# bkainz/fetalReconstruction

Measured on AMD Instinct MI355X. Metric: MVoxels/s per SR iteration (PSF fwd+back), 4-stack 1.0mm SVR, 1/2/4/8 GPU, higher is better.
Workload: dtype f32

## Files before the change

fetalreconstruction_amd/csrc/svr_cell.inc:

```

struct CellRec {
  short cx, cl, cz;
  unsigned short dead;
  float bx, by, bz;
  float f0, f1;
  uint32_t idx;
};
static_assert(sizeof(CellRec) == 32, "CellRec layout");

struct CellRun {
  uint32_t start, count;
  uint32_t cell, slice;
  short czmin, czmax;
  unsigned short n[4];
  int pad;
};
static_assert(sizeof(CellRun) == 32, "CellRun layout");

struct CellClass {
  int x0, l0;
  int ncx, ncl;
  int pfirst, plast;
  int ng;
  int cell_base;
// ... 384 lines not shown
  const uint32_t quad = item >> 10;
  const int ci = quad >= (uint32_t)ca.cls[1].cell_base ? 1 : 0;
  const CellClass &C = ca.cls[ci];
  const int P = C.pfirst + (int)(item & 1023u);
  const bool swap = ci == 0;
  const int vgy = swap ? vg.vz : vg.vy;
  const int lq = (int)quad - C.cell_base;
  const int ql = lq / C.ncx, qx = lq - ql * C.ncx;
  const int cx0 = C.x0 + qx * ca.CX, cl0 = C.l0 + ql * ca.CL;
  const int PL = ca.PL, PP = ca.PP;
  const bool idle = lane >= CH;
  const int slot = idle ? NSLOT - 1 : lane / SL, y = lane % SL;
  const float fyl = (float)(y - NC);
  const int lox = cx0 - NC, loy = cl0 - NC;
  f2 *pb = box + slot * PP - lox;
  for (int i = lane; i < NSLOT * PP; i += 64) box[i] = (f2){0.0f, 0.0f};
  __syncthreads();

  const uint32_t rfirst = ent.z, r1 = ent.w;
  uint32_t nreach = 0;
  for (uint32_t rb = rfirst; rb < r1; rb += 64) {
    CellRun Rl;
    Rl.start = Rl.count = Rl.slice = 0u;
    bool hit = false;
    if (rb + lane < r1) {
      Rl = ca.runs[rb + lane];
      hit = Rl.czmin - NC <= P && Rl.czmax + NH >= P;
    }
    unsigned long long todo = __ballot(hit);
    if (nparts > 1u) {
      const uint32_t ord = nreach + (uint32_t)__popcll(todo & ((1ull << lane) - 1ull));
      nreach += (uint32_t)__popcll(todo);
      todo = __ballot(hit && ord % nparts == rep);
    }
    const int mine = idle ? 0x7fffffff : NSLOT * y + slot;
    CellRec nrec;
    uint32_t npid = 0u;
    bool nact = false;
    nrec.f0 = nrec.f1 = 0.0f; nrec.cz = 0; nrec.dead = 0;
    auto request_run = [&](int rl) {
      const uint32_t st = (uint32_t)__builtin_amdgcn_readlane((int)Rl.start, rl), cn = (uint32_t)__builtin_amdgcn_readlane((int)Rl.count, rl);
      if ((uint32_t)mine < cn) {
        nrec = ca.recs[st + (uint32_t)mine];
        if (COEFF) npid = ca.pid[st + (uint32_t)mine];
        if (COEFF == 3) nact = ca.act[st + (uint32_t)mine] != 0;
      }
    };
    if (todo) request_run((int)__builtin_ctzll(todo));
    while (todo) {
      const int rl = (int)__builtin_ctzll(todo);
      todo &= todo - 1ull;
      const uint32_t sl = (uint32_t)__builtin_amdgcn_readlane((int)Rl.slice, rl);
      const uint32_t rstart = (uint32_t)__builtin_amdgcn_readlane((int)Rl.start, rl), rcount = (uint32_t)__builtin_amdgcn_readlane((int)Rl.count, rl);
      const SliceConst &S = a.sc[sl];
      const RowConst RC = load_row_const(S);
      for (uint32_t c0 = 0; c0 < rcount; c0 += CH) {
        CellRec r0;
        bool act0 = false;
        int pid0 = 0;
        if (c0 + (uint32_t)mine < rcount) {
          bool on0 = nact;
          if (c0 == 0) { r0 = nrec; pid0 = (int)npid; }
          else {
            r0 = ca.recs[rstart + c0 + (uint32_t)mine];
            if (COEFF) pid0 = (int)ca.pid[rstart + c0 + (uint32_t)mine];
            if (COEFF == 3) on0 = ca.act[rstart + c0 + (uint32_t)mine] != 0;
          }
          act0 = (COEFF == 3 ? on0 : (r0.f0 != 0.0f || r0.f1 != 0.0f)) && r0.cz - NC <= P && r0.cz + NH >= P;
        }
        if (c0 + CH >= rcount && todo) request_run((int)__builtin_ctzll(todo));
        if (ca.dbg == 2 && lane == 0) atomicAdd(ca.stats + 0, 1ull);
        if (!__any(act0)) continue;
        const bool dead0 = act0 && !PVR && ((r0.dead >> (P - r0.cz + NC)) & 1u);
        const int sh = SL * slot;
        unsigned ml = idle ? 0u : (unsigned)(__ballot(act0 && !dead0) >> sh) & ((1u << SL) - 1u);
        unsigned md = idle ? 0u : (unsigned)(__ballot(dead0) >> sh) & ((1u << SL) - 1u);
        if (ca.dbg == 2) {
          int mx = __popc(ml);
          for (int o = 16; o < 64; o <<= 1) mx = max(mx, __shfl_xor(mx, o, 64));
          if (y == 0 && !idle) { atomicAdd(ca.stats + 3, (unsigned long long)__popc(ml)); atomicAdd(ca.stats + 4, (unsigned long long)__popc(md)); }
          if (lane == 0) { atomicAdd(ca.stats + 1, 1ull); atomicAdd(ca.stats + 2, (unsigned long long)mx); }
        }
        const int w0a = (int)((unsigned short)r0.cx | ((unsigned)(unsigned short)r0.cl << 16));
        struct Unit { int cx, cy, cz; float bx, by, bz, f0, f1; int pid; };
        auto fetch = [&](int j) -> Unit {
          const int src = slot * SL + (j & 15);
          Unit u;
          const int w0 = __shfl(w0a, src, 64);
          u.cx = (int)(short)(w0 & 0xFFFF); u.cy = w0 >> 16;
          u.cz = __shfl((int)r0.cz, src, 64);
          u.f0 = __shfl(r0.f0, src, 64); u.f1 = __shfl(r0.f1, src, 64);
          u.pid = COEFF ? __shfl(pid0, src, 64) : 0;
          u.bx = u.by = u.bz = 0.0f;
          return u;
        };
        auto fetch_b = [&](int j, Unit &u) {
          const int src = slot * SL + (j & 15);
          u.bx = __shfl(r0.bx, src, 64); u.by = __shfl(r0.by, src, 64); u.bz = __shfl(r0.bz, src, 64);
        };
        if (ca.dbg == 0) {
          if (COEFF == 1) {
            constexpr int RING = SVR_CELL_RING;
            float4 ring[RING][NS / 4];
            Unit ru[RING];
            bool rv[RING];
            auto request = [&](Unit &u, bool &valid, float4 (&dst)[NS / 4]) {
              valid = ml != 0u;
              const int j = valid ? __builtin_ctz(ml) : 0;
              ml &= ml - 1u;
              u = fetch(j);
              if (valid) {
                const float4 *src = a.coeff + ((size_t)(uint32_t)u.pid * NS + (size_t)(P - u.cz + NC)) * (NS / 4 * 16) + (y < NS ? y : 0);
#pragma unroll
                for (int q = 0; q < NS / 4; ++q) dst[q] = load_stream(src + q * 16);
              }
            };
#pragma unroll
            for (int r3 = 0; r3 < RING; ++r3) request(ru[r3], rv[r3], ring[r3]);
            while (__any(rv[0])) {
#pragma unroll
              for (int r3 = 0; r3 < RING; ++r3) {
                if (!__any(rv[r3])) break;
                const Unit u = ru[r3];
                const bool valid = rv[r3];
                const int ay = u.cy + y - NC;
                const bool rowok = valid && y < NS && ay < vgy;
                const int rbx = rowok ? (ay - loy) * PL + u.cx - NC : lox;
                constexpr int PARTS = NS == 16 ? 2 : 1, PT = NS / PARTS;
                static_assert(PT % 4 == 0, "whole float4 per part");
                const f2 ff = (f2){u.f0, u.f1};
#pragma unroll
                for (int hq = 0; hq < PARTS; ++hq) {
                  f2 acc[PT];
#pragma unroll
                  for (int x = 0; x < PT; ++x) acc[x] = pb[rbx + hq * PT + x];
                  if (rowok) {
#pragma unroll
                    for (int q = 0; q < PT / 4; ++q) {
                      const float4 c = ring[r3][hq * (PT / 4) + q];
                      pb[rbx + hq * PT + 4 * q] = fma2(bc2(c.x), ff, acc[4 * q]);
                      pb[rbx + hq * PT + 4 * q + 1] = fma2(bc2(c.y), ff, acc[4 * q + 1]);
                      pb[rbx + hq * PT + 4 * q + 2] = fma2(bc2(c.z), ff, acc[4 * q + 2]);
                      pb[rbx + hq * PT + 4 * q + 3] = fma2(bc2(c.w), ff, acc[4 * q + 3]);
                    }
                  }
                }
                request(ru[r3], rv[r3], ring[r3]);
              }
            }
          } else {
            bool nvalid = ml != 0u;
            int jn = nvalid ? __builtin_ctz(ml) : 0;
            ml &= ml - 1u;
            Unit un = fetch(jn);
            fetch_b(jn, un);
            while (__any(nvalid)) {
              const bool valid = nvalid;
              const Unit u = un;
              nvalid = ml != 0u;
              jn = nvalid ? __builtin_ctz(ml) : 0;
              ml &= ml - 1u;
              un = fetch(jn);
              fetch_b(jn, un);
              const float fzu = (float)(P - u.cz);
              const int ay = u.cy + y - NC;
              const bool rowok = valid && y < NS && ay < vgy;
              const int rbx = rowok ? (ay - loy) * PL + u.cx - NC : lox;
              float out[NS];
              eval_row_t<NS, PVR, true, SVR_CELL_EVAL_H(NS)>(RC, u.bx, u.by, u.bz, swap ? fzu : fyl, swap ? fyl : fzu, out);
              if (COEFF == 3) {
                if (valid && y < NS) {
                  float4 *dstp = const_cast<float4 *>(a.coeff) + ((size_t)(uint32_t)u.pid * NS + (size_t)(P - u.cz + NC)) * (NS / 4 * 16) + y;
#pragma unroll
                  for (int q = 0; q < NS / 4; ++q) store_stream(dstp + q * 16, out[4 * q], out[4 * q + 1], out[4 * q + 2], out[4 * q + 3]);
                }
              }
              f2 acc[NS];
#pragma unroll
              for (int x = 0; x < NS; ++x) acc[x] = pb[rbx + x];
              if (rowok) {
                const f2 ff = (f2){u.f0, u.f1};
#pragma unroll
                for (int x = 0; x < NS; ++x) acc[x] = fma2(bc2(out[x]), ff, acc[x]);
#pragma unroll
                for (int x = 0; x < NS; ++x) pb[rbx + x] = acc[x];
              }
            }
          }
          if (!PVR) {
            while (__any(md != 0u)) {
              const bool va = md != 0u;
              const int ja = va ? __builtin_ctz(md) : 0;
              md &= md - 1u;
              const bool vb = md != 0u;
              const int jb = vb ? __builtin_ctz(md) : 0;
              md &= md - 1u;
              Unit Ra = fetch(ja), Rb = fetch(jb);
              fetch_b(ja, Ra); fetch_b(jb, Rb);
              const float fua = (float)(P - Ra.cz), fub = (float)(P - Rb.cz);
              const float fya = swap ? fua : fyl, fza = swap ? fyl : fua, fyb = swap ? fub : fyl, fzb = swap ? fyl : fub;
              const f2 rowx = (f2){__builtin_fmaf(RC.Lp[1], fya, __builtin_fmaf(RC.Lp[2], fza, Ra.bx)),
                                   __builtin_fmaf(RC.Lp[1], fyb, __builtin_fmaf(RC.Lp[2], fzb, Rb.bx))};
              const f2 rowy = (f2){__builtin_fmaf(RC.Lp[4], fya, __builtin_fmaf(RC.Lp[5], fza, Ra.by)),
                                   __builtin_fmaf(RC.Lp[4], fyb, __builtin_fmaf(RC.Lp[5], fzb, Rb.by))};
              const f2 rowz = (f2){__builtin_fmaf(RC.Lp[7], fya, __builtin_fmaf(RC.Lp[8], fza, Ra.bz)),
                                   __builtin_fmaf(RC.Lp[7], fyb, __builtin_fmaf(RC.Lp[8], fzb, Rb.bz))};
              f2 xs[1], ys[1], t0[1];
              xs[0] = fma2(bc2(RC.Lp[0]), bc2((float)(-NC)), rowx);
              ys[0] = fma2(bc2(RC.Lp[3]), bc2((float)(-NC)), rowy);
              eval_pairs_xyz<1, false>(RC, xs, ys, t0);
              const f2 v = t0[0] * gauss_first_tap2<NC>(RC, rowz);
              const int aya = Ra.cy + y - NC, ayb = Rb.cy + y - NC;
              if (va && aya < vgy) {
                f2 *q = pb + (aya - loy) * PL + Ra.cx - NC;
                *q = fma2(bc2(v.x), (f2){Ra.f0, Ra.f1}, *q);
              }
              if (vb && ayb < vgy) {
                f2 *q = pb + (ayb - loy) * PL + Rb.cx - NC;
                *q = fma2(bc2(v.y), (f2){Rb.f0, Rb.f1}, *q);
              }
            }
          }
        }
      }
    }
  }
  __syncthreads();
  f2 *dst = ca.stage + (size_t)bid * (size_t)PP;
  for (int i = lane; i < PP; i += 64) {
    f2 v = (box[i] + box[PP + i]) + (box[2 * PP + i] + box[3 * PP + i]);
    if (NSLOT == 5) v = v + box[4 * PP + i];
    dst[i] = v;
  }
  if (ca.trace && lane == 0) {
    unsigned hw, xcc;
    asm volatile("s_getreg_b32 %0, hwreg(HW_REG_HW_ID)" : "=s"(hw));
    asm volatile("s_getreg_b32 %0, hwreg(HW_REG_XCC_ID)" : "=s"(xcc));
    ca.trace[3 * (size_t)bid] = t_start;
    ca.trace[3 * (size_t)bid + 1] = __builtin_amdgcn_s_memrealtime();
    ca.trace[3 * (size_t)bid + 2] = (unsigned long long)hw | (unsigned long long)xcc << 32;
  }
}

__device__ __forceinline__ f2 combine_class(const CellArgs &ca, const CellClass &C, int c, int x, int y, int z, int NC, int NH, f2 acc) {
  const int Pv = c == 0 ? y : z, Lv = c == 0 ? z : y;
  const int pa = Pv > 0 ? Pv : min(C.pfirst, 0), pe = Pv > 0 ? Pv : 0;
  const int la = Lv > 0 ? Lv : min(C.l0 - NC, 0), le = Lv > 0 ? Lv : 0;
  const int xa = x > 0 ? x : min(C.x0 - NC, 0), xe = x > 0 ? x : 0;
  for (int Ps = max(pa, C.pfirst); Ps <= min(pe, C.plast); ++Ps) {
    const int g = Ps - C.pfirst;
    for (int Ls = la; Ls <= le; ++Ls) {
      const int jlo = max(-floordiv(-(Ls - C.l0 - NH - (ca.CL - 1)), ca.CL), 0);
      const int jhi = min(floordiv(Ls - C.l0 + NC, ca.CL), C.ncl * ca.QL - 1);
      for (int Xs = xa; Xs <= xe; ++Xs) {
        const int ilo = max(-floordiv(-(Xs - C.x0 - NH - (ca.CX - 1)), ca.CX), 0);
// ... 197 lines not shown
  const float fyl = (float)(y - NC);
  SlotSum<SL> ssum;
  ssum.init(lane);
  {
    const uint32_t sty = swap ? (uint32_t)(vg.vx * vg.vy) : (uint32_t)vg.vx, stz = swap ? (uint32_t)vg.vx : (uint32_t)(vg.vx * vg.vy);
    const uint32_t zoff = sat0(P) * stz;
    RowWalk w;
    w.init(lane, 64, PL);
    for (int i = lane; i < PP; i += 64, w.step()) {
      const int gx = w.x + lox, gy = w.y + loy;
      f2 v = (f2){0.0f, 0.0f};
      if (gx < vg.vx && gy < vgy) {
        const uint32_t vi = sat0(gx) + sat0(gy) * sty + zoff;
        if (G1) {
          v = (f2){1.0f, a.mask[vi] != 0.0f ? 1.0f : 0.0f};
        } else if (!PVR || a.volm) {
          const float2 t = a.volm[vi];
          v = (f2){t.x, t.y};
        } else {
          const float m = a.mask[vi] != 0.0f ? 1.0f : 0.0f;
          const int X = (int)sat0(gx), L = (int)sat0(gy), Z = (int)sat0(P);
          v = (f2){m != 0.0f ? pvr_tex(a.vol, vg, X, swap ? Z : L, swap ? L : Z) : 0.0f, m};
        }
      }
      box[i] = v;
    }
  }
  __syncthreads();
  const f2 *pb = box - lox;
  const float4 *stage = reinterpret_cast<const float4 *>(tile + 2 * ((PP + 1) & ~1)) + lane;
  const uint32_t stage_lds = COEFF == 2 ? (uint32_t)__builtin_amdgcn_readfirstlane((int)lds_addr_of(tile + 2 * ((PP + 1) & ~1))) : 0u;

  const uint32_t rfirst = ent.z, r1 = ent.w;
  uint32_t nreach = 0;
  for (uint32_t rb = rfirst; rb < r1; rb += 64) {
    CellRun Rl;
    Rl.start = Rl.count = Rl.slice = 0u;
    bool hit = false;
    if (rb + lane < r1) {
      Rl = ca.runs[rb + lane];
      hit = Rl.czmin - NC <= P && Rl.czmax + NH >= P;
    }
    unsigned long long todo = __ballot(hit);
    if (nparts > 1u) {
      const uint32_t ord = nreach + (uint32_t)__popcll(todo & ((1ull << lane) - 1ull));
      nreach += (uint32_t)__popcll(todo);
      todo = __ballot(hit && ord % nparts == rep);
    }
    const int mine = idle ? 0x7fffffff : NSLOT * y + slot;
    CellRec nrec;
    float ngf = 0.0f;
    uint32_t npid = 0u;
    nrec.cz = 0; nrec.dead = 0;
    auto request_run = [&](int rl) {
      const uint32_t st = (uint32_t)__builtin_amdgcn_readlane((int)Rl.start, rl), cn = (uint32_t)__builtin_amdgcn_readlane((int)Rl.count, rl);
      if ((uint32_t)mine < cn) { nrec = ca.recs[st + (uint32_t)mine]; ngf = G1 ? 1.0f : gf[st + (uint32_t)mine]; if (COEFF) npid = ca.pid[st + (uint32_t)mine]; }
    };
    if (todo) request_run((int)__builtin_ctzll(todo));
    while (todo) {
      const int rl = (int)__builtin_ctzll(todo);
      todo &= todo - 1ull;
      const uint32_t sl = (uint32_t)__builtin_amdgcn_readlane((int)Rl.slice, rl);
      const uint32_t rstart = (uint32_t)__builtin_amdgcn_readlane((int)Rl.start, rl), rcount = (uint32_t)__builtin_amdgcn_readlane((int)Rl.count, rl);
      const SliceConst &S = a.sc[sl];
      const RowConst RC = load_row_const(S);
      for (uint32_t c0 = 0; c0 < rcount; c0 += CH) {
        CellRec r0;
        float g0 = 0.0f;
        bool act0 = false;
        int pid0 = 0;
        if (c0 + (uint32_t)mine < rcount) {
          if (c0 == 0) { r0 = nrec; g0 = ngf; pid0 = (int)npid; }
          else { r0 = ca.recs[rstart + c0 + (uint32_t)mine]; g0 = G1 ? 1.0f : gf[rstart + c0 + (uint32_t)mine]; if (COEFF) pid0 = (int)ca.pid[rstart + c0 + (uint32_t)mine]; }
          act0 = g0 != 0.0f && r0.cz - NC <= P && r0.cz + NH >= P;
        }
        if (c0 + CH >= rcount && todo) request_run((int)__builtin_ctzll(todo));
        if (!__any(act0)) continue;
        const bool dead0 = act0 && !PVR && ((r0.dead >> (P - r0.cz + NC)) & 1u);
        const int sh = SL * slot;
        unsigned ml = idle ? 0u : (unsigned)(__ballot(act0 && !dead0) >> sh) & ((1u << SL) - 1u);
        unsigned md = idle ? 0u : (unsigned)(__ballot(dead0) >> sh) & ((1u << SL) - 1u);
        const int w0a = (int)((unsigned short)r0.cx | ((unsigned)(unsigned short)r0.cl << 16));
        const uint32_t myrec = rstart + c0 + (uint32_t)mine;
        struct Unit { int cx, cy, cz; float bx, by, bz; uint32_t rec; int pid; };
        auto fetch = [&](int j) -> Unit {
          const int src = slot * SL + (j & 15);
          Unit u;
          const int w0 = __shfl(w0a, src, 64);
          u.cx = (int)(short)(w0 & 0xFFFF); u.cy = w0 >> 16;
          u.cz = __shfl((int)r0.cz, src, 64);
          u.bx = __shfl(r0.bx, src, 64); u.by = __shfl(r0.by, src, 64); u.bz = __shfl(r0.bz, src, 64);
          u.rec = (uint32_t)__shfl((int)myrec, src, 64);
          u.pid = COEFF ? __shfl(pid0, src, 64) : 0;
          return u;
        };
        if (COEFF == 2) {
          static_assert(COEFF != 2 || NS == 16, "the landing stages are laid out for support 16");
          constexpr int DD = SVR_CELL_DMA_DEPTH, HQ = NS / 4;
          unsigned mli = ml;
          int s_issue = 0, s_use = 0;
          auto issue = [&]() -> bool {
            const bool vi = mli != 0u;
            if (!__any(vi)) return false;
            const int j = vi ? __builtin_ctz(mli) : 0;
            mli &= mli - 1u;
            const int src = slot * SL + (j & 15);
            const int pid = __shfl(pid0, src, 64), czk = __shfl((int)r0.cz, src, 64);
            const float4 *srcp = vi ? a.coeff + ((size_t)(uint32_t)pid * NS + (size_t)(P - czk + NC)) * (HQ * 16) + y : a.coeff + lane;
            const uint32_t dst = stage_lds + (uint32_t)s_issue * (HQ * 1024u);
#pragma unroll
            for (int q = 0; q < HQ; ++q) glds16(srcp + q * 16, dst + q * 1024u);
            s_issue = s_issue + 1 == DD ? 0 : s_issue + 1;
            return true;
          };
#pragma unroll
          for (int k = 0; k < DD - 1; ++k) issue();
          bool nvalid = ml != 0u;
          int jn = nvalid ? __builtin_ctz(ml) : 0;
          ml &= ml - 1u;
          Unit un = fetch(jn);
          while (__any(nvalid)) {
            const bool ahead = issue();
            const bool valid = nvalid;
            const Unit u = un;
            nvalid = ml != 0u;
            jn = nvalid ? __builtin_ctz(ml) : 0;
            ml &= ml - 1u;
            un = fetch(jn);
            const int ay = u.cy + y - NC;
            const bool rowok = valid && ay < vgy;
            f2 acc = (f2){0.0f, 0.0f};
            {
              const f2 *q = pb + (rowok ? (ay - loy) * PL + u.cx - NC : lox);
              if (ahead) glds_wait<(DD - 1) * HQ>(); else glds_wait<0>();
              const float4 *st = stage + s_use * (HQ * 64);
              s_use = s_use + 1 == DD ? 0 : s_use + 1;
#pragma unroll
              for (int qq = 0; qq < HQ; ++qq) {
                const float4 c = st[qq * 64];
                acc = fma2(bc2(c.x), q[4 * qq], acc);
                acc = fma2(bc2(c.y), q[4 * qq + 1], acc);
                acc = fma2(bc2(c.z), q[4 * qq + 2], acc);
                acc = fma2(bc2(c.w), q[4 * qq + 3], acc);
              }
            }
            if (!rowok) acc = (f2){0.0f, 0.0f};
            acc.x = ssum.sum(acc.x); acc.y = ssum.sum(acc.y);
            if (valid && y == 0) part[(size_t)(P - u.cz + NC) * npart + u.rec] = acc;
          }
        } else if (COEFF == 1) {
          constexpr int RING = SVR_CELL_RING;
          float4 ring[RING][NS / 4];
          Unit ru[RING];
          bool rv[RING];
          auto request = [&](Unit &u, bool &valid, float4 (&dst)[NS / 4]) {
            valid = ml != 0u;
            const int j = valid ? __builtin_ctz(ml) : 0;
            ml &= ml - 1u;
            u = fetch(j);
            if (valid) {
              const float4 *src = a.coeff + ((size_t)(uint32_t)u.pid * NS + (size_t)(P - u.cz + NC)) * (NS / 4 * 16) + (y < NS ? y : 0);
#pragma unroll
              for (int q = 0; q < NS / 4; ++q) dst[q] = load_stream(src + q * 16);
            }
          };
#pragma unroll
          for (int r3 = 0; r3 < RING; ++r3) request(ru[r3], rv[r3], ring[r3]);
          while (__any(rv[0])) {
#pragma unroll
            for (int r3 = 0; r3 < RING; ++r3) {
              if (!__any(rv[r3])) break;
              const Unit u = ru[r3];
              const bool valid = rv[r3];
              const int ay = u.cy + y - NC;
              const bool rowok = valid && y < NS && ay < vgy;
              f2 acc = (f2){0.0f, 0.0f};
              {
                const f2 *q = pb + (rowok ? (ay - loy) * PL + u.cx - NC : lox);
#pragma unroll
                for (int qq = 0; qq < NS / 4; ++qq) {
                  const float4 c = ring[r3][qq];
                  acc = fma2(bc2(c.x), q[4 * qq], acc);
                  acc = fma2(bc2(c.y), q[4 * qq + 1], acc);
                  acc = fma2(bc2(c.z), q[4 * qq + 2], acc);
                  acc = fma2(bc2(c.w), q[4 * qq + 3], acc);
                }
              }
              request(ru[r3], rv[r3], ring[r3]);
              if (!rowok) acc = (f2){0.0f, 0.0f};
              acc.x = ssum.sum(acc.x); acc.y = ssum.sum(acc.y);
              if (valid && y == 0) part[(size_t)(P - u.cz + NC) * npart + u.rec] = acc;
            }
          }
        }
        if (COEFF == 0 || COEFF == 3) {
        bool nvalid = ml != 0u;
        int jn = nvalid ? __builtin_ctz(ml) : 0;
        ml &= ml - 1u;
        Unit un = fetch(jn);
        while (__any(nvalid)) {
          const bool valid = nvalid;
          const Unit u = un;
          nvalid = ml != 0u;
          jn = nvalid ? __builtin_ctz(ml) : 0;
          ml &= ml - 1u;
          un = fetch(jn);
          const float fzu = (float)(P - u.cz);
          const int ay = u.cy + y - NC;
          const bool rowok = valid && y < NS && ay < vgy;
          float out[NS];
          eval_row_t<NS, PVR, true, SVR_CELL_EVAL_H_FWD(NS)>(RC, u.bx, u.by, u.bz, swap ? fzu : fyl, swap ? fyl : fzu, out);
          if (COEFF == 3) {
            if (valid && y < NS) {
              float4 *dstp = const_cast<float4 *>(a.coeff) + ((size_t)(uint32_t)u.pid * NS + (size_t)(P - u.cz + NC)) * (NS / 4 * 16) + y;
#pragma unroll
              for (int q = 0; q < NS / 4; ++q) store_stream(dstp + q * 16, out[4 * q], out[4 * q + 1], out[4 * q + 2], out[4 * q + 3]);
            }
          }
          f2 acc = (f2){0.0f, 0.0f};
          double accd = 0.0;
          bool hit = false;
          {
            const f2 *q = pb + (rowok ? (ay - loy) * PL + u.cx - NC : lox);
            f2 v[NS];
#pragma unroll
            for (int x = 0; x < NS; ++x) v[x] = q[x];
#pragma unroll
            for (int x = 0; x < NS; ++x) {
              if (G1) {
                accd += (double)(out[x] * v[x].x);
                hit = hit | ((v[x].y != 0.0f) & (__float_as_uint(out[x]) != 0x80000000u));
              } else {
                acc = fma2(bc2(out[x]), v[x], acc);
              }
            }
          }
          if (G1) {
            if (!rowok) { accd = 0.0; hit = false; }
            accd = ssum.sum(accd);
            const bool anyhit = idle ? false : (((uint32_t)(__ballot(hit) >> (SL * slot)) & ((1u << SL) - 1u)) != 0u);
            if (valid && y == 0) partd[(size_t)(P - u.cz + NC) * npart + u.rec] = anyhit ? -accd : accd;
          } else {
            if (!rowok) acc = (f2){0.0f, 0.0f};
            acc.x = ssum.sum(acc.x); acc.y = ssum.sum(acc.y);
            if (valid && y == 0) part[(size_t)(P - u.cz + NC) * npart + u.rec] = acc;
          }
        }
        }
        if (!PVR) {
          while (__any(md != 0u)) {
            const bool va = md != 0u;
            const int ja = va ? __builtin_ctz(md) : 0;
            md &= md - 1u;
            const bool vb = md != 0u;
            const int jb = vb ? __builtin_ctz(md) : 0;
            md &= md - 1u;
            const Unit Ra = fetch(ja), Rb = fetch(jb);
            const float fua = (float)(P - Ra.cz), fub = (float)(P - Rb.cz);
            const float fya = swap ? fua : fyl, fza = swap ? fyl : fua, fyb = swap ? fub : fyl, fzb = swap ? fyl : fub;
            const f2 rowx = (f2){__builtin_fmaf(RC.Lp[1], fya, __builtin_fmaf(RC.Lp[2], fza, Ra.bx)),
                                 __builtin_fmaf(RC.Lp[1], fyb, __builtin_fmaf(RC.Lp[2], fzb, Rb.bx))};
            const f2 rowy = (f2){__builtin_fmaf(RC.Lp[4], fya, __builtin_fmaf(RC.Lp[5], fza, Ra.by)),
                                 __builtin_fmaf(RC.Lp[4], fyb, __builtin_fmaf(RC.Lp[5], fzb, Rb.by))};
            const f2 rowz = (f2){__builtin_fmaf(RC.Lp[7], fya, __builtin_fmaf(RC.Lp[8], fza, Ra.bz)),
                                 __builtin_fmaf(RC.Lp[7], fyb, __builtin_fmaf(RC.Lp[8], fzb, Rb.bz))};
            f2 xs[1], ys[1], t0[1];
            xs[0] = fma2(bc2(RC.Lp[0]), bc2((float)(-NC)), rowx);
            ys[0] = fma2(bc2(RC.Lp[3]), bc2((float)(-NC)), rowy);
            eval_pairs_xyz<1, false>(RC, xs, ys, t0);
            const f2 v = t0[0] * gauss_first_tap2<NC>(RC, rowz);
            const int aya = Ra.cy + y - NC, ayb = Rb.cy + y - NC;
            f2 wa = (f2){0.0f, 0.0f}, wb = (f2){0.0f, 0.0f};
            if (va && aya < vgy) wa = pb[(aya - loy) * PL + Ra.cx - NC];
            if (vb && ayb < vgy) wb = pb[(ayb - loy) * PL + Rb.cx - NC];
            f2 acca = bc2(v.x) * wa, accb = bc2(v.y) * wb;
            if (G1) {
              double da = row_sum16((double)acca.x), db = row_sum16((double)accb.x);
              const bool anya = ((uint32_t)(__ballot(wa.y != 0.0f) >> (16 * slot)) & 0xFFFFu) != 0u;
              const bool anyb = ((uint32_t)(__ballot(wb.y != 0.0f) >> (16 * slot)) & 0xFFFFu) != 0u;
              if (y == 0) {
                if (va) partd[(size_t)(P - Ra.cz + NC) * npart + Ra.rec] = anya ? -da : da;
                if (vb) partd[(size_t)(P - Rb.cz + NC) * npart + Rb.rec] = anyb ? -db : db;
              }
            } else {
              acca.x = row_sum16(acca.x); acca.y = row_sum16(acca.y);
              accb.x = row_sum16(accb.x); accb.y = row_sum16(accb.y);
              if (y == 0) {
                if (va) part[(size_t)(P - Ra.cz + NC) * npart + Ra.rec] = acca;
                if (vb) part[(size_t)(P - Rb.cz + NC) * npart + Rb.rec] = accb;
              }
            }
          }
        }
      }
    }
  }
}
// ... 540 lines not shown
```

fetalreconstruction_amd/csrc/svr_hip.hip:

```cpp
#include <hip/hip_runtime.h>
#include <float.h>
#include <limits.h>
#include <math.h>
#include <stdint.h>
#include <stdio.h>
#include <string.h>

#include <algorithm>
#include <chrono>
#include <string>
#include <vector>

#include "../../include/svr_hip.h"

int svr_sort_keys_u64(void *tmp, size_t *tmp_bytes, const uint64_t *keys_in, uint64_t *keys_out, size_t n, int end_bit, hipStream_t stream);
int svr_inclusive_sum_u32(void *tmp, size_t *tmp_bytes, const uint32_t *in, uint32_t *out, size_t n, hipStream_t stream);

#define SVR_STEP 0.0001f
#define PSF_SUPPORT 16
#define PSF_CENTRE 7
#define PSF_EPS_F 0.00001f
#define LDS_ROW 20
#define WAVES_PER_BLOCK 4
#define CHUNK_PIX 2048
// ... 18 lines not shown
  float I2W[12];
  float T[12];
  float A[12];
  float Lp[9];
  float dim[3];
  float kx, ky, inv2s2;
  float dd, w;
  int own;
  float invD;
  float pad[9];
};
static_assert(sizeof(SliceConst) == 256, "SliceConst layout");

struct VolGeom {
  int vx, vy, vz;
  float W2I[12];
  float c0[3];
  int pvr;
};

__host__ __device__ __forceinline__ float canon_exp_neg(float a) {
  const float LOG2E = 1.442695040888963407359924681001892137426645954152985934135449406931f;
  const float L2U = 0.693145751953125f;
  const float L2L = 1.428606765330187045e-06f;
  float d = -a;
  float q = __builtin_rintf(d * LOG2E);
  float s = __builtin_fmaf(q, -L2U, d);
  s = __builtin_fmaf(q, -L2L, s);
  float u = 0.000198527617612853646278381f;
  u = __builtin_fmaf(u, s, 0.00139304355252534151077271f);
  u = __builtin_fmaf(u, s, 0.00833336077630519866943359f);
  u = __builtin_fmaf(u, s, 0.0416664853692054748535156f);
  u = __builtin_fmaf(u, s, 0.166666671633720397949219f);
  u = __builtin_fmaf(u, s, 0.5f);
  u = __builtin_fmaf(s * s, u, s) + 1.0f;
  float r = ldexpf(u, (int)q);
  return (a > 87.0f) ? 0.0f : r;
}
__device__ __forceinline__ float wave_sum(float v) {
#pragma unroll
  for (int o = 32; o > 0; o >>= 1) v += __shfl_xor(v, o, 64);
  return v;
}
__device__ __forceinline__ double wave_sum(double v) {
#pragma unroll
  for (int o = 32; o > 0; o >>= 1) v += __shfl_xor(v, o, 64);
  return v;
}

__device__ __forceinline__ void matvec3(const float *M, float x, float y, float z, float &a,
                                        float &b, float &c) {
  a = M[0] * x + M[1] * y + M[2] * z + M[3];
  b = M[4] * x + M[5] * y + M[6] * z + M[7];
  c = M[8] * x + M[9] * y + M[10] * z + M[11];
}

enum { MODE_GAUSS = 0, MODE_FWD = 1, MODE_BACK = 2, MODE_BIAS = 3 };

struct PsfArgs {
  const SliceConst *sc;
  VolGeom vg;
  int sx, sy;
  const uint32_t *list;
  uint32_t n;
  const float *slices;
  const float *mask;
  float *psf_sums;
  const float *scales;
  const float *bias;
  const unsigned char *flag;
  unsigned char *flag_out;
  const unsigned char *spx;
  float *recon, *volw;
  int *voxcount;
  const float *vol;
  const float2 *volm;
  float *simslices, *simweights;
  unsigned char *siminside;
  unsigned char *slice_inside;
  const float *weights, *slice_weights;
  float *addon, *cmap;
  const float4 *coeff;
  const uint32_t *coeff_id;
};

struct PixelState {
  int cxi, cyi, czi;
  float bx, by, bz;
};

__device__ __forceinline__ int clampi(float f) {
  f = fminf(fmaxf(f, -1048576.0f), 1048576.0f);
  return (int)f;
}

__device__ __forceinline__ PixelState pixel_setup(const SliceConst &S, const VolGeom &vg, int px,
                                                  int py) {
  PixelState P;
  float wx, wy, wz, tx, ty, tz, vx_, vy_, vz_;
  matvec3(S.I2W, (float)px, (float)py, 0.0f, wx, wy, wz);
  matvec3(S.T, wx, wy, wz, tx, ty, tz);
  matvec3(vg.W2I, tx, ty, tz, vx_, vy_, vz_);
  float cx = roundf(vx_), cy = roundf(vy_), cz = roundf(vz_);
  P.cxi = clampi(cx); P.cyi = clampi(cy); P.czi = clampi(cz);
  double d0 = (double)S.A[0] * cx + (double)S.A[1] * cy + (double)S.A[2] * cz + (double)S.A[3] - (double)(float)px;
  double d1 = (double)S.A[4] * cx + (double)S.A[5] * cy + (double)S.A[6] * cz + (double)S.A[7] - (double)(float)py;
  double d2 = (double)S.A[8] * cx + (double)S.A[9] * cy + (double)S.A[10] * cz + (double)S.A[11] - 0.0;
  P.bx = (float)((d0 * S.dim[0] - vg.c0[0]) * S.kx);
  P.by = (float)((d1 * S.dim[1] - vg.c0[1]) * S.ky);
  P.bz = vg.pvr ? (float)(d2 * S.dim[2] / 2.5 - vg.c0[2]) : (float)(d2 * S.dim[2] - vg.c0[2]);
  return P;
}

struct RowConst {
  float Lp[9];
  float inv2s2;
  float dd, w;
  float invD;
};
__device__ __forceinline__ float uniform_f(float v) {
  return __builtin_bit_cast(float, __builtin_amdgcn_readfirstlane(__builtin_bit_cast(int, v)));
}
__device__ __forceinline__ RowConst load_row_const(const SliceConst &S) {
  RowConst R;
#pragma unroll
  for (int i = 0; i < 9; ++i) R.Lp[i] = S.Lp[i];
  R.inv2s2 = uniform_f(S.inv2s2);
  R.dd = uniform_f(S.dd);
  R.w = uniform_f(S.w);
  R.invD = uniform_f(S.invD);
  return R;
}

typedef float f2 __attribute__((ext_vector_type(2)));
__device__ __forceinline__ f2 fma2(f2 a, f2 b, f2 c) { return __builtin_elementwise_fma(a, b, c); }
__device__ __forceinline__ f2 bc2(float c) { return (f2)(c); }

__device__ __forceinline__ f2 exp_neg2(f2 a) {
  const f2 t = -a * bc2(1.442695040888963407359924681001892137426645954152985934135449406931f);
  const f2 k = (f2){__builtin_rintf(t.x), __builtin_rintf(t.y)};
  f2 r = fma2(k, bc2(-0.693145751953125f), -a);
  r = fma2(k, bc2(-1.428606765330187045e-06f), r);
  f2 s = fma2(bc2(0.000198527617612853646278381f), r, bc2(0.00139304355252534151077271f));
  s = fma2(s, r, bc2(0.00833336077630519866943359f));
  s = fma2(s, r, bc2(0.0416664853692054748535156f));
  s = fma2(s, r, bc2(0.166666671633720397949219f));
  s = fma2(s, r, bc2(0.5f));
  s = fma2(r * r, s, r) + bc2(1.0f);
  s = (f2){ldexpf(s.x, (int)k.x), ldexpf(s.y, (int)k.y)};
  return (f2){(a.x > 87.0f) ? 0.0f : s.x, (a.y > 87.0f) ? 0.0f : s.y};
}

#define GAUSS_AMAX 60.0f
__device__ __attribute__((noinline)) f2 gauss_direct2(float dz, float rowz, float inv2s2, float j, bool keep, f2 g) {
  const f2 z = fma2(bc2(dz), (f2){-j, 1.0f + j}, bc2(rowz));
  const f2 e = exp_neg2((z * z) * bc2(inv2s2));
  return keep ? g : e;
}
struct GaussStep {
  f2 g, r;
  bool ok;
};
__device__ __forceinline__ GaussStep gauss_start(const RowConst S, float rowz) {
  const f2 zc = fma2(bc2(S.Lp[6]), (f2){0.0f, 1.0f}, bc2(rowz));
  const f2 ac = (zc * zc) * bc2(S.inv2s2);
  const f2 t = fma2(((f2){-2.0f, 2.0f}) * zc, bc2(S.Lp[6]), bc2(S.dd)) * bc2(S.inv2s2);
// ... 382 lines not shown
  if (SVR_XCD_RUN <= 0) return b;
  constexpr uint32_t R = SVR_XCD_RUN > 0 ? SVR_XCD_RUN : 1, G = 8u * R;
  const uint32_t base = b / G * G;
  if (base + G > n) return b;
  const uint32_t q = b - base;
  return base + (q & 7u) * R + (q >> 3);
}


struct PixelRec {
  int cx, cy, cz;
  float bx, by, bz;
  float f0, f1;
};

#define SLOT_MAXP 48
struct RowWalk {
  int x, y, tx, ty, P;
  __device__ __forceinline__ void init(int i0, int stride, int P_) {
    P = P_;
    y = i0 / P; x = i0 - y * P;
    ty = stride / P; tx = stride - ty * P;
  }
  __device__ __forceinline__ void step() {
    x += tx; y += ty;
    if (x >= P) { x -= P; ++y; }
  }
};

__device__ __forceinline__ bool unit_is_dead(const RowConst S, float bx, float by, float bz, int F, float fo) {
  const bool f1 = F == 1;
  const float LxF = f1 ? S.Lp[1] : S.Lp[2], LxG = f1 ? S.Lp[2] : S.Lp[1];
  const float LyF = f1 ? S.Lp[4] : S.Lp[5], LyG = f1 ? S.Lp[5] : S.Lp[4];
  const float LzF = f1 ? S.Lp[7] : S.Lp[8], LzG = f1 ? S.Lp[8] : S.Lp[7];
  const float lo_ = (float)(-PSF_CENTRE), hi_ = (float)(PSF_SUPPORT - 1 - PSF_CENTRE);
  const float c = __builtin_fmaf(LzF, fo, bz);
  const float zlo = c + fminf(S.Lp[6] * lo_, S.Lp[6] * hi_) + fminf(LzG * lo_, LzG * hi_);
  const float zhi = c + fmaxf(S.Lp[6] * lo_, S.Lp[6] * hi_) + fmaxf(LzG * lo_, LzG * hi_);
  if (!(zlo > 0.0f || zhi < 0.0f)) return false;
  const float zmin = fminf(fabsf(zlo), fabsf(zhi)) * 0.999f - 1e-4f;
  if (!(zmin > 0.0f && (zmin * zmin) * S.inv2s2 > SVR_DEAD_THR)) return false;
  if (S.invD == 0.0f) return false;
  const float cx = __builtin_fmaf(LxF, fo, bx), cy = __builtin_fmaf(LyF, fo, by);
  const float ox = (cy * LxG - cx * LyG) * S.invD, og = (cx * S.Lp[3] - cy * S.Lp[0]) * S.invD;
  if (!(fabsf(ox) < 64.0f && fabsf(og) < 64.0f)) return true;
  const float fx0 = floorf(ox), fg0 = floorf(og);
  bool zero = false;
#pragma unroll
  for (int j = 0; j < 4; ++j) {
    const float fx = fx0 + (float)(j & 1), fg = fg0 + (float)(j >> 1);
    const float fy = f1 ? fo : fg, fz = f1 ? fg : fo;
    const float xs = __builtin_fmaf(S.Lp[0], fx, __builtin_fmaf(S.Lp[1], fy, __builtin_fmaf(S.Lp[2], fz, bx)));
    const float ys = __builtin_fmaf(S.Lp[3], fx, __builtin_fmaf(S.Lp[4], fy, __builtin_fmaf(S.Lp[5], fz, by)));
    zero = zero || __builtin_fmaf(ys, ys, xs * xs) == 0.0f;
  }
  return !zero;
}

typedef float nt_f4 __attribute__((ext_vector_type(4)));
__device__ __forceinline__ float4 load_stream(const float4 *p) {
  const nt_f4 v = __builtin_nontemporal_load(reinterpret_cast<const nt_f4 *>(p));
  return make_float4(v.x, v.y, v.z, v.w);
}

__device__ __forceinline__ void glds16(const void *gsrc, uint32_t lds_dst) {
  unsigned keep;
  asm volatile("s_mov_b32 %0, m0\n\ts_mov_b32 m0, %2\n\ts_nop 0\n\tglobal_load_lds_dwordx4 %1, off nt\n\ts_mov_b32 m0, %0"
               : "=&s"(keep) : "v"(gsrc), "s"(lds_dst) : "memory");
}
template <int N>
__device__ __forceinline__ void glds_wait() { asm volatile("s_waitcnt vmcnt(%0)" :: "n"(N) : "memory"); }
__device__ __forceinline__ uint32_t lds_addr_of(const void *p) { return (uint32_t)(uintptr_t)p; }

#ifndef SVR_COEFF_STORE_NT
#define SVR_COEFF_STORE_NT 1
#endif
__device__ __forceinline__ void store_stream(float4 *p, float a, float b, float c, float d) {
#if SVR_COEFF_STORE_NT
  __builtin_nontemporal_store((nt_f4){a, b, c, d}, reinterpret_cast<nt_f4 *>(p));
#else
  *p = make_float4(a, b, c, d);
#endif
}
template <int NS, bool PVR>
__global__ __launch_bounds__(256) void k_coeff_build(PsfArgs a, float4 *coeff, uint32_t *coeff_id, uint32_t base) {
  constexpr int NC = (NS - 1) / 2, QUADS = NS / 4;
  static_assert(NS % 4 == 0 && NS <= 16, "tap quads, one row per lane of a 16-lane slot");
  const uint32_t wl = blockIdx.x * 4u + (threadIdx.x >> 6);
  if (wl >= a.n) return;
  const int lane = threadIdx.x & 63;
  const uint32_t idx = a.list[wl];
  const uint32_t w = base + wl;
  const uint32_t n2 = (uint32_t)(a.sx * a.sy);
  const uint32_t sl = idx / n2, rem = idx - sl * n2;
  const int py = (int)(rem / (uint32_t)a.sx), px = (int)(rem - (uint32_t)py * (uint32_t)a.sx);
  const SliceConst &S = a.sc[sl];
  const PixelState P = pixel_setup(S, a.vg, px, py);
  const RowConst RC = load_row_const(S);
  const bool swap = S.own == 1;
  const int F = swap ? 1 : 2;
  if (lane == 0) coeff_id[idx] = w;
  const int slot = lane >> 4, y = lane & 15;
  const float fyl = (float)(y - NC);
  for (int g = 0; 4 * g < NS; ++g) {
    const int u = 4 * g + slot;
    const float fu = (float)(u - NC);
    const bool dead = !PVR && unit_is_dead(RC, P.bx, P.by, P.bz, F, fu);
    if (__all(dead)) continue;
    float out[NS];
    eval_row_t<NS, PVR, true>(RC, P.bx, P.by, P.bz, swap ? fu : fyl, swap ? fyl : fu, out);
    if (!dead && u < NS && y < NS) {
      float4 *dst = coeff + ((size_t)w * NS + u) * (QUADS * 16) + y;
#pragma unroll
      for (int q = 0; q < QUADS; ++q) store_stream(dst + q * 16, out[4 * q], out[4 * q + 1], out[4 * q + 2], out[4 * q + 3]);
    }
  }
}



__device__ __forceinline__ float pvr_tex(const float *vol, const VolGeom &vg, int X, int Y, int Z) {
  float v = 0.0f;
#pragma unroll
  for (int dz = -1; dz <= 0; ++dz)
#pragma unroll
    for (int dy = -1; dy <= 0; ++dy)
#pragma unroll
      for (int dx = -1; dx <= 0; ++dx) {
        const int x = X + dx, y = Y + dy, z = Z + dz;
        const float t = (x >= 0 && y >= 0 && z >= 0) ? vol[(size_t)x + (size_t)y * vg.vx + (size_t)z * vg.vx * vg.vy] : 0.0f;
        v += 0.125f * t;
      }
  return v;
}

template <int N> __device__ __forceinline__ int row_shl_i(int v) {
  return __builtin_amdgcn_update_dpp(0, v, 0x100 + N, 0xF, 0xF, true);
}
template <int N> __device__ __forceinline__ float row_shl_f(float v) {
  return __builtin_bit_cast(float, row_shl_i<N>(__builtin_bit_cast(int, v)));
}
template <int N> __device__ __forceinline__ double row_shl_d(double v) {
  const unsigned long long b = __builtin_bit_cast(unsigned long long, v);
  const unsigned lo = (unsigned)row_shl_i<N>((int)(unsigned)b), hi = (unsigned)row_shl_i<N>((int)(unsigned)(b >> 32));
  return __builtin_bit_cast(double, ((unsigned long long)hi << 32) | lo);
}
__device__ __forceinline__ float row_sum16(float v) {
  v += row_shl_f<8>(v); v += row_shl_f<4>(v); v += row_shl_f<2>(v); v += row_shl_f<1>(v);
  return v;
}
__device__ __forceinline__ double row_sum16(double v) {
  v += row_shl_d<8>(v); v += row_shl_d<4>(v); v += row_shl_d<2>(v); v += row_shl_d<1>(v);
  return v;
}
#include "svr_tile.inc"

#define PVR_N 12
#define PVR_CENTRE 5

#define MODE_GAUSS2 4
template <int MODE>
__device__ __forceinline__ void pvr_pixel(const PsfArgs &a, uint32_t idx, int lane) {
  const uint32_t n2 = (uint32_t)(a.sx * a.sy);
  const uint32_t sl = idx / n2;
  const uint32_t rem = idx - sl * n2;
  const int py = (int)(rem / (uint32_t)a.sx);
  const int px = (int)(rem - (uint32_t)py * (uint32_t)a.sx);
  const SliceConst &S = a.sc[sl];
  const VolGeom &vg = a.vg;
  const PixelState P = pixel_setup(S, vg, px, py);
  const RowConst RC = load_row_const(S);
  float s = a.slices[idx] * a.scales[sl];
  float sume;
  if (MODE == MODE_GAUSS) {
    double acc = 0.0;
    const bool spx_ok = !a.spx || a.spx[(size_t)sl * 4096 + px + 64 * py] == '1';
    if (spx_ok) {
      for (int p = 0; p < 3; ++p) {
        const int r = p * 64 + lane;
        const bool valid = r < PVR_N * PVR_N;
        const int z = r / PVR_N, y = r - z * PVR_N;
        float out[PVR_N];
        eval_row_t<PVR_N, true>(RC, P.bx, P.by, P.bz, (float)(y - PVR_CENTRE), (float)(z - PVR_CENTRE), out);
        const uint32_t az = sat0(P.czi + z - PVR_CENTRE), ay = sat0(P.cyi + y - PVR_CENTRE);
        const bool rowin = valid && az < (uint32_t)vg.vz && ay < (uint32_t)vg.vy;
#pragma unroll
        for (int x = 0; x < PVR_N; ++x) {
          const uint32_t ax = sat0(P.cxi + x - PVR_CENTRE);
          acc += (rowin && ax < (uint32_t)vg.vx && !(out[x] < 0.0f)) ? (double)out[x] : 0.0;
        }
      }
    }
    sume = (float)wave_sum(acc);
    if (!((sume > 0.00001f) || (sume != sume))) return;
// ... 138 lines not shown
  int reg_mode = 1;
  bool prep_pending = false;
  bool cmap_from_scatter = false;
  float2 *d_volm = nullptr;
  bool have_mask = false;
  int mbox_lo[3] = {0, 0, 0}, mbox_hi[3] = {-1, -1, -1};
  bool mbox_valid = false;
  float *d_pair_pack = nullptr;
  size_t pair_pack_cap = 0;

  uint32_t sx = 0, sy = 0, ns = 0;
  size_t np = 0;
  float *d_slices = nullptr, *d_weights = nullptr, *d_simslices = nullptr, *d_simweights = nullptr,
        *d_psf_sums = nullptr;
  unsigned char *d_siminside = nullptr;
  int *d_voxcount = nullptr;
  bool have_slices = false;
  bool have_sim = false;
  bool sem_weights_current = false;
  float *d_scales = nullptr, *d_slice_weights = nullptr, *d_scales_host_copy = nullptr,
        *d_tmp_ns = nullptr;
  unsigned char *d_slice_inside = nullptr;
  std::vector<float> h_slice_weights;
  bool have_scales = false;
  static constexpr int UP_SLOTS = 4;
  float *h_up = nullptr;
  hipEvent_t up_ev[UP_SLOTS] = {nullptr, nullptr, nullptr, nullptr};
  bool up_busy[UP_SLOTS] = {false, false, false, false};
  int up_next = 0;
  std::vector<float> mir_scales, mir_slice_weights, mir_scales_copy;
  unsigned char *h_down = nullptr;
  size_t down_cap = 0, down_used = 0;
  struct DownItem { void *dst; size_t off, bytes; };
  std::vector<DownItem> down_items;
  float *d_em = nullptr;

  std::vector<float> slice_dims;
  std::vector<uint32_t> stack_sizes;
  std::vector<float> mI2W, mW2I, mT, mTinv;
  float reconI2W[16], reconW2I[16];
  float psf_c0[3] = {0, 0, 0};
  float quality_factor = 1.0f;
  bool have_dims = false, have_mats = false, have_psf = false, sc_dirty = true;
  SliceConst *d_sc = nullptr;

  uint32_t *d_active = nullptr, *d_psf_list = nullptr, *d_counter = nullptr, *d_tiles = nullptr,
           *d_tiles_fb = nullptr;
  uint32_t n_active = 0, n_psf = 0, n_tiles = 0;
  int tiles_x = 0, tiles_y = 0, tile_w = 4, tile_h = 4;
  int reg_blind = 4;
  int reg_red_threads = 0;
  int reg_batch = 1;
  int pvr_reg_levels = 3, pvr_reg_steps = 4, pvr_reg_iterations = 20;
  bool psf_list_valid = false;
  unsigned char *d_gauss_flag = nullptr;
  uint32_t *d_tiles_tmp = nullptr;
  size_t tiles_tmp_cap = 0;
  int gauss_mode = 1;
  uint32_t *d_tiles_fwd = nullptr;
  uint32_t n_tiles_fwd = 0;
  bool tiles_back_valid = false, tiles_fwd_valid = false;
  int fwd_tw = 4, fwd_th = 4, fwd_tiles_x = 0, fwd_tiles_y = 0;
  int fwd_unit_cap = 9300;
  int fwd_mode = 2;
  bool fwd_tile_user = false, tile_user = false;
  int pvr = 0;
  int pvr_mode = 1;
  unsigned char *d_spx = nullptr;
  int back_mode = 5;
  int tile_cap = 0;
  int n_cu = 0;
  uint32_t n_tiles_fb = 0;
  uint32_t n_tiles_fb8 = 0;
  uint64_t fallbacks[4] = {0, 0, 0, 0};
  void note_fallback(int kind, const char *what) {
    if (!fallbacks[kind]++) fprintf(stderr, "svr: %s -- counted in svr_fallbacks()[%d]\n", what, kind);
  }
  uint32_t *d_tiles_fb2 = nullptr;
  bool wave_cap_user = false;
  bool back_mode_user = false;
  bool fwd_mode_user = false;
  bool sr_no_wait = false;
  float4 *d_coeff = nullptr;
  uint32_t *d_coeff_id = nullptr;
  uint32_t *d_coeff_order = nullptr;
  size_t coeff_order_cap = 0;
  size_t coeff_cap = 0;
  CoeffState coeff_state = COEFF_NONE;
  int coeff_mode = 1;
  bool legacy_ok = false;
  bool coeff_user = false;
  int coeff_lazy = 1;
  const uint32_t *coeff_list = nullptr;
  bool coeff_ids_valid = false;
  int wave_groups = 1, wave_cap = 2096;

  double *d_partial = nullptr, *d_per_slice = nullptr, *d_out = nullptr;
  double *d_em_all = nullptr;
  size_t em_all_cap = 0;
  int chunks = 0;

  float *d_bias = nullptr, *d_wb = nullptr, *d_wr = nullptr, *d_buffer = nullptr;
  float *d_bias_vol = nullptr, *d_volume_weights = nullptr, *d_maskC = nullptr, *d_mbuf = nullptr;
  float mask_sigma_bias = 12.0f;
  int bias_mode = 1;
  int bias_corrections = 0, bias_normalisations = 0;
  int bias_scatters = 0, bias_scatters_on_cells = 0;
  int last_bias_bx = -1, last_tail_lds = -1, last_tail_rows = -1, last_tail_bxy = -1, last_tail_bxz = -1;
  int last_reg_zc = -1, last_reg_chunks = -1;
  bool maskC_valid = false;

  short *d_reg_targets = nullptr, *d_reg_source = nullptr;
  short *d_pyr_full[2] = {nullptr, nullptr}, *d_pyr_a = nullptr, *d_pyr_b = nullptr;
  size_t pyr_full_cap[2] = {0, 0}, pyr_work_cap = 0;
  void *d_pyr_meta = nullptr;
  size_t pyr_meta_cap = 0;
  int *d_ncc_idx = nullptr;
  double *d_ncc_m = nullptr;
  long long *d_ncc_s = nullptr;
  size_t ncc_cap = 0;
  unsigned char *d_nmi_io = nullptr;
  size_t nmi_cap = 0;
  std::vector<unsigned char> nmi_staging;
  double *d_nmi_terms = nullptr;
  size_t nmi_terms_n = 0;
  unsigned *d_nmi_merge = nullptr;
  size_t nmi_slots = 0;
  float *d_mot_x = nullptr;
  double *d_mot_partial = nullptr, *d_mot_g = nullptr;
  double *d_qual_partial = nullptr, *d_qual_sums = nullptr;
  int last_quality_chunks = -1;
  int reg_tx = 0, reg_ty = 0, reg_n = 0;
  uint32_t reg_vx = 0, reg_vy = 0, reg_vz = 0;

  RegState *reg = nullptr;

  SliceEm *sem = nullptr;
  SlabPlan *slab = nullptr;
  bool vol_clean[2] = {false, false};
  CellState *cell = nullptr;
  CellState *cell_g = nullptr;
  int *d_cellc = nullptr;
  size_t cellc_cap = 0;
  uint32_t cellc_n = 0;
  bool cellc_valid = false;
  int cellc_range[16] = {0};
  int cell_w = 0, cell_h = 0, cell_gw = 0, cell_gh = 0;
  int cell_order = 1;
  int cell_combine = 2;
  int cell_balance = 0;
  int cell_split = 1, cell_qx = 1, cell_band = 3;

  bool timers = false;
  struct TimedSpan { int which; hipEvent_t a, b; };
  std::vector<hipEvent_t> ev_free;
  std::vector<TimedSpan> ev_pending;
  hipEvent_t ev_open = nullptr;
  double t_ms[SVR_T_COUNT] = {0};
  long t_n[SVR_T_COUNT] = {0};

  float *recon() { return recon_cur; }
  float *volw() { return d_recon_volw + nv; }
  float *addon() { return d_addon_cmap; }
  float *cmap() { return d_addon_cmap + nv; }
};

// ... 193 lines not shown
int build_tile_list(svr_ctx *ctx, const float *psf_sums, const unsigned char *flag, int tiles_x, int tiles_y, int tw, int th, uint32_t *tiles,
                    uint32_t *counter) {
  const uint64_t total64 = (uint64_t)tiles_x * tiles_y * ctx->ns;
  if (total64 >= (1ull << 32)) return fail(ctx, SVR_E_ARG, "more than 2^32 candidate tiles");
  return in_pieces((uint32_t)total64, 64, [&](uint32_t off, uint32_t cnt) {
    hipLaunchKernelGGL(k_build_tiles, dim3(nblk(cnt, 16)), dim3(1024), 0, ctx->stream, ctx->d_slices, psf_sums, flag, (int)ctx->sx, (int)ctx->sy,
                       (int)ctx->ns, tiles_x, tiles_y, tw, th, tiles, counter, (const unsigned char *)nullptr, 0, off, off + cnt);
    KCHK("k_build_tiles");
    return (int)SVR_OK;
  });
}

int build_list(svr_ctx *ctx, bool with_psf) {
  HIPCHK(hipMemsetAsync(ctx->d_counter, 0, sizeof(uint32_t), ctx->stream));
  uint32_t *list = with_psf ? ctx->d_psf_list : ctx->d_active;
  hipLaunchKernelGGL(k_compact, dim3(std::min(nblk(ctx->np, 1024), 4096u)), dim3(1024), 0, ctx->stream, ctx->d_slices,
                     with_psf ? ctx->d_psf_sums : (const float *)nullptr, (uint32_t)ctx->np, list, ctx->d_counter);
  KCHK("k_compact");
  uint32_t n = 0;
  HIPCHK(hipMemcpyAsync(&n, ctx->d_counter, sizeof(n), hipMemcpyDeviceToHost, ctx->stream));
  HIPCHK(hipStreamSynchronize(ctx->stream));
  if (with_psf) {
    ctx->n_psf = n;
    ctx->psf_list_valid = true;
    ctx->tiles_back_valid = ctx->tiles_fwd_valid = false;
  } else {
    ctx->n_active = n;
  }
  return SVR_OK;
}
int ensure_psf_list(svr_ctx *ctx);
int ensure_tiles_back(svr_ctx *ctx) {
  int r = ensure_psf_list(ctx);
  if (r || ctx->tiles_back_valid) return r;
  uint32_t n = 0;
  HIPCHK(hipMemsetAsync(ctx->d_counter, 0, sizeof(uint32_t), ctx->stream));
  if ((r = build_tile_list(ctx, ctx->d_psf_sums, nullptr, ctx->tiles_x, ctx->tiles_y, ctx->tile_w, ctx->tile_h, ctx->d_tiles, ctx->d_counter))) return r;
  HIPCHK(hipMemcpyAsync(&n, ctx->d_counter, sizeof(n), hipMemcpyDeviceToHost, ctx->stream));
  HIPCHK(hipStreamSynchronize(ctx->stream));
  ctx->n_tiles = n;
  ctx->tiles_back_valid = true;
  return SVR_OK;
}
int ensure_tiles_fwd(svr_ctx *ctx) {
  int r = ensure_psf_list(ctx);
  if (r || ctx->tiles_fwd_valid) return r;
  uint32_t n = 0;
  free_dev(ctx->d_tiles_fwd);
  ctx->fwd_tiles_x = (int)((ctx->sx + ctx->fwd_tw - 1) / ctx->fwd_tw);
  ctx->fwd_tiles_y = (int)((ctx->sy + ctx->fwd_th - 1) / ctx->fwd_th);
  const uint32_t total_f = (uint32_t)ctx->fwd_tiles_x * ctx->fwd_tiles_y * ctx->ns;
  HIPCHK(hipMalloc(&ctx->d_tiles_fwd, (size_t)total_f * sizeof(uint32_t)));
  HIPCHK(hipMemsetAsync(ctx->d_counter, 0, sizeof(uint32_t), ctx->stream));
  if ((r = build_tile_list(ctx, ctx->d_psf_sums, nullptr, ctx->fwd_tiles_x, ctx->fwd_tiles_y, ctx->fwd_tw, ctx->fwd_th, ctx->d_tiles_fwd, ctx->d_counter))) return r;
  HIPCHK(hipMemcpyAsync(&n, ctx->d_counter, sizeof(n), hipMemcpyDeviceToHost, ctx->stream));
  HIPCHK(hipStreamSynchronize(ctx->stream));
  ctx->n_tiles_fwd = n;
  ctx->tiles_fwd_valid = true;
  return SVR_OK;
}

PsfArgs make_args(svr_ctx *ctx) {
  PsfArgs a;
  memset(&a, 0, sizeof(a));
  a.sc = ctx->d_sc;
  a.vg.vx = (int)ctx->vx; a.vg.vy = (int)ctx->vy; a.vg.vz = (int)ctx->vz;
  memcpy(a.vg.W2I, ctx->reconW2I, 12 * sizeof(float));
  memcpy(a.vg.c0, ctx->psf_c0, 3 * sizeof(float));
  a.vg.pvr = ctx->pvr;
  a.spx = ctx->d_spx;
  a.sx = (int)ctx->sx; a.sy = (int)ctx->sy;
  a.slices = ctx->d_slices; a.mask = ctx->d_mask; a.psf_sums = ctx->d_psf_sums;
  a.scales = ctx->d_scales;
  a.bias = ctx->disable_bias ? nullptr : ctx->d_bias;
  a.recon = ctx->recon(); a.volw = ctx->volw(); a.voxcount = ctx->d_voxcount;
  a.vol = ctx->recon(); a.simslices = ctx->d_simslices; a.simweights = ctx->d_simweights;
  a.siminside = ctx->d_siminside;
  a.slice_inside = ctx->d_slice_inside;
  a.weights = ctx->d_weights; a.slice_weights = ctx->d_slice_weights;
  a.addon = ctx->addon(); a.cmap = ctx->cmap();
  return a;
}

void give_coeff(const svr_ctx *ctx, PsfArgs &a) { a.coeff = ctx->d_coeff; a.coeff_id = ctx->d_coeff_id; }

int ensure_bias_buffers(svr_ctx *ctx) {
  if (ctx->disable_bias) return SVR_OK;
  if (ctx->np && !ctx->d_bias) {
    const size_t fb = ctx->np * sizeof(float);
    HIPCHK(hipMalloc(&ctx->d_bias, fb)); HIPCHK(hipMalloc(&ctx->d_wb, fb));
    HIPCHK(hipMalloc(&ctx->d_wr, fb)); HIPCHK(hipMalloc(&ctx->d_buffer, fb));
    HIPCHK(hipMemsetAsync(ctx->d_bias, 0, fb, ctx->stream));
    HIPCHK(hipMemsetAsync(ctx->d_wb, 0, fb, ctx->stream));
    HIPCHK(hipMemsetAsync(ctx->d_wr, 0, fb, ctx->stream));
    HIPCHK(hipMemsetAsync(ctx->d_buffer, 0, fb, ctx->stream));
  }
  if (ctx->nv && !ctx->d_bias_vol) {
    const size_t vb = ctx->nv * sizeof(float);
    HIPCHK(hipMalloc(&ctx->d_bias_vol, vb)); HIPCHK(hipMalloc(&ctx->d_volume_weights, vb));
    HIPCHK(hipMalloc(&ctx->d_maskC, vb)); HIPCHK(hipMalloc(&ctx->d_mbuf, vb));
    HIPCHK(hipMemsetAsync(ctx->d_bias_vol, 0, vb, ctx->stream));
    HIPCHK(hipMemsetAsync(ctx->d_volume_weights, 0, vb, ctx->stream));
  }
  if (ctx->nv && ctx->have_mask && !ctx->maskC_valid) {
    const size_t vb = ctx->nv * sizeof(float);
    const dim3 grid((ctx->vx + 63) / 64, (ctx->vy + 3) / 4, ctx->vz);
    HIPCHK(hipMemcpyAsync(ctx->d_maskC, ctx->d_mask, vb, hipMemcpyDeviceToDevice, ctx->stream));
    HIPCHK(hipMemsetAsync(ctx->d_mbuf, 0, vb, ctx->stream));
    hipLaunchKernelGGL(k_gauss_conv3d, grid, dim3(256), 0, ctx->stream, ctx->d_maskC, ctx->d_mbuf, ctx->mask_sigma_bias, 0,
                       ctx->vdim[0], (int)ctx->vx, (int)ctx->vy, (int)ctx->vz);
    hipLaunchKernelGGL(k_gauss_conv3d, grid, dim3(256), 0, ctx->stream, ctx->d_mbuf, ctx->d_maskC, ctx->mask_sigma_bias, 1,
                       ctx->vdim[1], (int)ctx->vx, (int)ctx->vy, (int)ctx->vz);
    hipLaunchKernelGGL(k_gauss_conv3d, grid, dim3(256), 0, ctx->stream, ctx->d_maskC, ctx->d_mbuf, ctx->mask_sigma_bias, 2,
                       ctx->vdim[2], (int)ctx->vx, (int)ctx->vy, (int)ctx->vz);
    KCHK("k_gauss_conv3d(mask)");
    HIPCHK(hipMemcpyAsync(ctx->d_maskC, ctx->d_mbuf, vb, hipMemcpyDeviceToDevice, ctx->stream));
    HIPCHK(hipStreamSynchronize(ctx->stream));
    ctx->maskC_valid = true;
  }
  return SVR_OK;
}

int ready(svr_ctx *ctx) {
  NEED(ctx->nv > 0, "reconstruction volume not initialised");
  NEED(ctx->have_mask, "mask not set");
  NEED(ctx->have_slices, "slices not filled");
  NEED(ctx->have_scales, "scale vector not set");
  NEED(ctx->have_psf, "generatePSFVolume not called");
  int r = ensure_bias_buffers(ctx);
  if (r) return r;
  return prepare_slice_consts(ctx);
}

template <bool GAUSS1>
void launch_fwd_unit(svr_ctx *ctx, const PsfArgs &a, TileArgs ta, size_t lds) {
  constexpr uint32_t PIECE_MAX = 1u << 22;
  static_assert((uint64_t)PIECE_MAX * FWDU_WAVES * 64 < (1ull << 32), "a piece must fit one dispatch");
  const char *env = getenv("SVR_FWD_PIECE");
  const uint32_t PIECE = env && atol(env) > 0 ? (uint32_t)std::min<long>(atol(env), PIECE_MAX) : PIECE_MAX;
  const uint32_t *tiles = ta.tiles;
  const uint32_t total = ta.ntiles;
  for (uint32_t off = 0; off < total; off += PIECE) {
    ta.tiles = tiles + off;
    ta.ntiles = std::min(PIECE, total - off);
    const dim3 grid(ta.ntiles), block(FWDU_WAVES * 64);
    if (ctx->pvr && a.coeff) hipLaunchKernelGGL((fwd_unit_kernel<GAUSS1, PVR_N, true, true>), grid, block, lds, ctx->stream, a, ta);
    else if (ctx->pvr) hipLaunchKernelGGL((fwd_unit_kernel<GAUSS1, PVR_N, true>), grid, block, lds, ctx->stream, a, ta);
    else if (a.coeff) hipLaunchKernelGGL((fwd_unit_kernel<GAUSS1, PSF_SUPPORT, false, true>), grid, block, lds, ctx->stream, a, ta);
    else hipLaunchKernelGGL((fwd_unit_kernel<GAUSS1>), grid, block, lds, ctx->stream, a, ta);
  }
}

int ensure_psf_list(svr_ctx *ctx) {
  if (!ctx->psf_list_valid) return build_list(ctx, true);
  return SVR_OK;
}

int coeff_order(svr_ctx *ctx, uint32_t n_active, const uint32_t **list);
__global__ void k_coeff_ids(const uint32_t *list, uint32_t n, uint32_t *coeff_id) {
  const uint32_t i = blockIdx.x * blockDim.x + threadIdx.x;
  if (i < n) coeff_id[list[i]] = i;
}
bool coeff_lazy_ok(const svr_ctx *ctx) { return ctx->coeff_lazy && !ctx->pvr && ctx->fwd_mode == 2; }
bool coeff_lazy_pending(const svr_ctx *ctx) { return ctx->coeff_mode && ctx->coeff_state == COEFF_NONE && coeff_lazy_ok(ctx); }
bool table_holds(const svr_ctx *ctx, CoeffState need) { return ctx->coeff_mode && ctx->coeff_state >= need; }
int coeff_prepare(svr_ctx *ctx, const uint32_t **list) {
  const size_t npx = ctx->n_active;
  if (npx > ctx->coeff_cap) {
    free_dev(ctx->d_coeff);
    ctx->coeff_cap = 0;
    size_t fr = 0, tot = 0;
    const size_t per_px = ctx->pvr ? (size_t)PVR_N * (PVR_N / 4) * 16 : (size_t)PSF_SUPPORT * (PSF_SUPPORT / 4) * 16;
    const size_t bytes = npx * per_px * sizeof(float4);
    const char *cap_gb = getenv("SVR_COEFF_MAX_GB");
    const bool over = cap_gb && (double)bytes > atof(cap_gb) * 1073741824.0;
    const size_t bias_later = ctx->disable_bias ? 0 : (ctx->d_bias ? 0 : 4 * ctx->np * sizeof(float)) + (ctx->d_bias_vol ? 0 : 4 * ctx->nv * sizeof(float));
    if (over || hipMemGetInfo(&fr, &tot) != hipSuccess || bytes + bias_later + (size_t(2) << 30) > fr || hipMalloc(&ctx->d_coeff, bytes) != hipSuccess) {
      (void)hipGetLastError();
      ctx->d_coeff = nullptr;
      ctx->coeff_mode = 0;
      return SVR_OK;
    }
    ctx->coeff_cap = npx;
  }
  if (!ctx->d_coeff_id) HIPCHK(hipMalloc(&ctx->d_coeff_id, ctx->np * sizeof(uint32_t)));
  if (ctx->coeff_ids_valid && ctx->coeff_list) { *list = ctx->coeff_list; return SVR_OK; }
  *list = ctx->d_active;
  if (!getenv("SVR_COEFF_UNSORTED")) {
    const int r = coeff_order(ctx, (uint32_t)npx, list);
    if (r) return r;
  }
  ctx->coeff_list = *list;
  return SVR_OK;
}
int ensure_coeff(svr_ctx *ctx) {
  if (!ctx->coeff_mode || ctx->coeff_state != COEFF_NONE) return SVR_OK;
  const size_t npx = ctx->n_active;
  if (!npx) return SVR_OK;
  PsfArgs a = make_args(ctx);
  a.n = (uint32_t)npx;
  { const int r = coeff_prepare(ctx, &a.list); if (r) return r; }
  if (!ctx->coeff_mode) return SVR_OK;
  ScopedTimer tb(ctx, SVR_T_COEFF_BUILD);
  {
    const int rr = pixel_list_in_pieces(a, [&](const PsfArgs &ap, uint32_t off) {
      if (ctx->pvr) hipLaunchKernelGGL((k_coeff_build<PVR_N, true>), dim3(nblk(ap.n, 4)), dim3(256), 0, ctx->stream, ap, ctx->d_coeff, ctx->d_coeff_id, off);
      else hipLaunchKernelGGL((k_coeff_build<PSF_SUPPORT, false>), dim3(nblk(ap.n, 4)), dim3(256), 0, ctx->stream, ap, ctx->d_coeff, ctx->d_coeff_id, off);
      KCHK("k_coeff_build");
      return (int)SVR_OK;
    });
    if (rr) return rr;
  }
  tb.stop();
  ctx->coeff_state = COEFF_FULL;
  if (!ctx->coeff_ids_valid) invalidate(ctx, CH_TABLE_IDS);
  ctx->coeff_ids_valid = true;
  return SVR_OK;
}
int coeff_begin_store(svr_ctx *ctx, bool *store) {
  *store = false;
  if (!coeff_lazy_pending(ctx) || !ctx->n_active) return SVR_OK;
  const uint32_t *order = nullptr;
  int r = coeff_prepare(ctx, &order);
  if (r) return r;
  if (!ctx->coeff_mode) return SVR_OK;
  if (!ctx->coeff_ids_valid) {
    hipLaunchKernelGGL(k_coeff_ids, dim3(nblk(ctx->n_active)), dim3(256), 0, ctx->stream, order, (uint32_t)ctx->n_active, ctx->d_coeff_id);
    KCHK("k_coeff_ids");
    invalidate(ctx, CH_TABLE_IDS);
    ctx->coeff_ids_valid = true;
  }
  *store = true;
  return SVR_OK;
}

int launch_slot(svr_ctx *ctx, bool pvr, const PsfArgs &a, const TileArgs &ta_, uint32_t *fb, uint32_t *cnt) {
  const size_t lds = (size_t)ta_.cap * 2 * sizeof(float);
  return in_pieces(ta_.ntiles, 8 * 64, [&](uint32_t off, uint32_t cntp) {
    TileArgs ta = ta_;
    ta.tiles = ta_.tiles + off; ta.ntiles = cntp;
    if (pvr) hipLaunchKernelGGL((back_slot_kernel<8, PVR_N, true>), dim3(ta.ntiles), dim3(8 * 64), lds, ctx->stream, a, ta, fb, cnt);
    else hipLaunchKernelGGL(back_slot_kernel<8>, dim3(ta.ntiles), dim3(8 * 64), lds, ctx->stream, a, ta, fb, cnt);
    KCHK("back_slot_kernel");
    return (int)SVR_OK;
  });
}
int launch_scatter(svr_ctx *ctx, int level, const PsfArgs &a_, const uint32_t *tiles, uint32_t n, int mode_last) {
  PsfArgs a = a_;
  TileArgs ta;
  ta.tiles_x = ctx->tiles_x; ta.tiles_y = ctx->tiles_y; ta.tw = ctx->tile_w; ta.th = ctx->tile_h; ta.gauss = mode_last == MODE_GAUSS2;
  const bool pvr = ctx->pvr != 0;
  uint32_t *cnt = ctx->d_counter;
  HIPCHK(hipMemsetAsync(cnt, 0, 2 * sizeof(uint32_t), ctx->stream));
  ctx->n_tiles_fb8 = ctx->n_tiles_fb = 0;
  if (!n) return SVR_OK;
  int r;
  uint32_t nfb[2] = {0, 0};
  const uint32_t *cur = tiles;
  uint32_t ncur = n;
  if (level >= 4) {
    ta.tiles = cur; ta.ntiles = ncur; ta.cap = std::min(ctx->wave_cap, ctx->tile_cap);
    const size_t lds = (size_t)ta.cap * 2 * sizeof(float);
    {
      const TileArgs ta1 = ta;
      r = in_pieces(ncur, 64u * (uint32_t)ctx->wave_groups, [&](uint32_t off, uint32_t cntp) {
        TileArgs tp = ta1;
        tp.tiles = ta1.tiles + off; tp.ntiles = cntp;
        const dim3 grid(cntp * (uint32_t)ctx->wave_groups);
        if (pvr && a.coeff) hipLaunchKernelGGL((back_wave_kernel<PVR_N, true, true>), grid, dim3(64), lds, ctx->stream, a, tp, ctx->wave_groups, ctx->d_tiles_fb, cnt);
        else if (pvr) hipLaunchKernelGGL((back_wave_kernel<PVR_N, true>), grid, dim3(64), lds, ctx->stream, a, tp, ctx->wave_groups, ctx->d_tiles_fb, cnt);
        else if (a.coeff) hipLaunchKernelGGL((back_wave_kernel<PSF_SUPPORT, false, true>), grid, dim3(64), lds, ctx->stream, a, tp, ctx->wave_groups, ctx->d_tiles_fb, cnt);
        else hipLaunchKernelGGL(back_wave_kernel<>, grid, dim3(64), lds, ctx->stream, a, tp, ctx->wave_groups, ctx->d_tiles_fb, cnt);
        return (int)SVR_OK;
      });
      if (r) return r;
    }
    KCHK("back_wave_kernel");
    HIPCHK(hipMemcpyAsync(nfb, cnt, sizeof(nfb), hipMemcpyDeviceToHost, ctx->stream));
    HIPCHK(hipStreamSynchronize(ctx->stream));
    cur = ctx->d_tiles_fb; ncur = nfb[0];
    if (ncur && a.coeff && ta.cap < 3696) {
      HIPCHK(hipMemsetAsync(cnt, 0, sizeof(uint32_t), ctx->stream));
      ta.tiles = cur; ta.ntiles = ncur; ta.cap = std::min(3696, ctx->tile_cap);
      if (pvr) hipLaunchKernelGGL((back_wave_kernel<PVR_N, true, true>), dim3(ncur * (uint32_t)ctx->wave_groups), dim3(64), (size_t)ta.cap * 2 * sizeof(float),
                                  ctx->stream, a, ta, ctx->wave_groups, ctx->d_tiles_fb2, cnt);
      else hipLaunchKernelGGL((back_wave_kernel<PSF_SUPPORT, false, true>), dim3(ncur * (uint32_t)ctx->wave_groups), dim3(64), (size_t)ta.cap * 2 * sizeof(float),
                              ctx->stream, a, ta, ctx->wave_groups, ctx->d_tiles_fb2, cnt);
      KCHK("back_wave_kernel (large box)");
      HIPCHK(hipMemcpyAsync(nfb, cnt, sizeof(nfb), hipMemcpyDeviceToHost, ctx->stream));
      HIPCHK(hipStreamSynchronize(ctx->stream));
      cur = ctx->d_tiles_fb2; ncur = nfb[0];
      if (ncur) {
        HIPCHK(hipMemcpyAsync(ctx->d_tiles_fb, ctx->d_tiles_fb2, (size_t)ncur * sizeof(uint32_t), hipMemcpyDeviceToDevice, ctx->stream));
        cur = ctx->d_tiles_fb;
      }
    }
    ctx->n_tiles_fb8 = ncur;
    ctx->fallbacks[3] += ncur;
  }
  if (ncur && level >= 3) {
    ta.tiles = cur; ta.ntiles = ncur; ta.cap = ctx->tile_cap;
    if ((r = launch_slot(ctx, pvr, a, ta, ctx->d_tiles_fb2, cnt + 1))) return r;
    HIPCHK(hipMemcpyAsync(nfb, cnt, sizeof(nfb), hipMemcpyDeviceToHost, ctx->stream));
    HIPCHK(hipStreamSynchronize(ctx->stream));
    cur = ctx->d_tiles_fb2; ncur = nfb[1];
  }
  if (level >= 3) ctx->n_tiles_fb = ncur;
  if (ncur) {
    ta.tiles = cur; ta.ntiles = ncur; ta.cap = ctx->tile_cap;
    if (pvr && mode_last == MODE_GAUSS2) { a.recon = a.addon; a.volw = a.cmap; }
    const TileArgs ta0 = ta;
    r = in_pieces(ncur, pvr ? WAVES_PER_BLOCK * 64 : TILE_WAVES * 64, [&](uint32_t off, uint32_t cntp) {
      ta.tiles = ta0.tiles + off; ta.ntiles = cntp;
      if (pvr) {
        if (mode_last == MODE_GAUSS2) hipLaunchKernelGGL(pvr_tiles_kernel<MODE_GAUSS2>, dim3(cntp), dim3(WAVES_PER_BLOCK * 64), 0, ctx->stream, a, ta);
        else hipLaunchKernelGGL(pvr_tiles_kernel<MODE_BACK>, dim3(cntp), dim3(WAVES_PER_BLOCK * 64), 0, ctx->stream, a, ta);
      } else {
        hipLaunchKernelGGL(back_tiled_kernel, dim3(cntp), dim3(TILE_WAVES * 64), (size_t)ctx->tile_cap * 2 * sizeof(float), ctx->stream, a, ta);
      }
      KCHK("scatter (last resort)");
      return (int)SVR_OK;
    });
    if (r) return r;
  }
  return SVR_OK;
}

#include "svr_cell.inc"
#include "svr_slab.inc"

void invalidate(svr_ctx *ctx, unsigned ch) {
  if (ch & CH_SLICE_GEOMETRY) ctx->sc_dirty = true;
  if (ch & (CH_SLICE_PIXELS | CH_PSF_SUMS | CH_TILE_SHAPE)) ctx->psf_list_valid = false;
  if (ch & (CH_TAPS | CH_SLICE_PIXELS | CH_VOLUME_GRID | CH_TABLE | CH_TABLE_OFF)) ctx->coeff_state = COEFF_NONE;
  if ((ch & CH_PSF_SUMS) && ctx->coeff_state == COEFF_PSF) ctx->coeff_state = COEFF_NONE;
  if (ch & CH_TABLE_OFF) { free_dev(ctx->d_coeff); ctx->coeff_cap = 0; }
  const bool cells = ch & (CH_TAPS | CH_SLICE_PIXELS | CH_VOLUME_GRID | CH_CELL_SHAPE | CH_TABLE_OFF);
  if (cells) ctx->cellc_valid = ctx->coeff_ids_valid = false;
  for (CellState *cs : {ctx->cell, ctx->cell_g}) {
    if (!cs) continue;
    if (cells) cs->valid = false;
    if (cells || (ch & CH_PSF_SUMS)) cs->gf_valid = false;
    if (cells || (ch & CH_TABLE_IDS)) cs->pid_valid = false;
  }
  if (ch & (CH_VOLUME_GRID | CH_MASK)) { ctx->vol_clean[0] = ctx->vol_clean[1] = false; if (ctx->slab) ctx->slab->valid = false; }
  if (ch & CH_MASK) ctx->mbox_valid = false;
  if (ch & (CH_VOLUME_GRID | CH_MASK_BLUR)) ctx->maskC_valid = false;
  if (ch & CH_VOLUME_VALUES) ctx->vol_clean[ctx->recon_cur == ctx->d_recon_new ? 1 : 0] = false;
  if (ch & (CH_VOLUME_GRID | CH_SCATTER_TARGETS)) ctx->cmap_from_scatter = false;
}

double pixel_density(const svr_ctx *ctx) {
  double d = 1.0;
  if (ctx->slice_dims.size() >= 3 && ctx->slice_dims[0] > 0 && ctx->slice_dims[1] > 0)
    d = (double)ctx->vdim[0] * ctx->vdim[1] / ((double)ctx->slice_dims[0] * ctx->slice_dims[1]);
  return d;
}
void tile_shape_rule(const svr_ctx *ctx, bool table, int &w, int &h) {
  const double d = pixel_density(ctx);
  if (ctx->pvr) { w = 8; h = 4; }
  else if (table && d < 0.65) { w = 6; h = 5; }
  else { w = 6; h = 4; }
}
int set_scatter_tile(svr_ctx *ctx, int w, int h) {
  ctx->tile_w = w; ctx->tile_h = h;
  if (!ctx->np) return SVR_OK;
  free_dev(ctx->d_tiles); free_dev(ctx->d_tiles_fb); free_dev(ctx->d_tiles_fb2);
  ctx->tiles_x = (int)((ctx->sx + w - 1) / w);
  ctx->tiles_y = (int)((ctx->sy + h - 1) / h);
  const size_t nb = (size_t)ctx->tiles_x * ctx->tiles_y * ctx->ns * sizeof(uint32_t);
  HIPCHK(hipMalloc(&ctx->d_tiles, nb));
  HIPCHK(hipMalloc(&ctx->d_tiles_fb, nb));
  HIPCHK(hipMalloc(&ctx->d_tiles_fb2, nb));
  invalidate(ctx, CH_TILE_SHAPE);
  return SVR_OK;
}

enum Family {
  FAM_CELLS,
  FAM_TILES,
  FAM_PIXELS,
};
enum Pass { PASS_GAUSS1, PASS_GAUSS2, PASS_FORWARD, PASS_BACK, PASS_BIAS };
struct PassPath {
  Family family;
  int scatter_level;
  bool may_stream_table;
  bool table_on_cells;
};
PassPath pass_path(const svr_ctx *ctx, Pass pass) {
  const bool pvr = ctx->pvr != 0;
  const bool pvr_units = ctx->pvr_mode == 1;
  PassPath p = {FAM_PIXELS, 0, false, false};
  switch (pass) {
    case PASS_GAUSS1:
    case PASS_GAUSS2:
      if (ctx->gauss_mode != 1 || (pvr && !pvr_units)) break;
      p.may_stream_table = true;
      if (pass == PASS_GAUSS1) p.family = ctx->fwd_mode == 2 ? FAM_CELLS : FAM_TILES;
      else p.family = ctx->back_mode == 5 ? FAM_CELLS : FAM_TILES;
      p.scatter_level = pvr ? 4 : std::min(4, std::max(1, ctx->back_mode));
      break;
    case PASS_FORWARD:
      if (pvr ? !pvr_units : ctx->fwd_mode < 1) break;
      p.may_stream_table = true;
      p.family = ctx->fwd_mode == 2 ? FAM_CELLS : FAM_TILES;
      if (pvr) {
        int sw, sh, gw, gh;
        cell_sizes(ctx, sw, sh, gw, gh);
        p.table_on_cells = gw * gh >= 96 || ctx->fwd_mode_user;
      } else {
        p.table_on_cells = ctx->fwd_mode_user || pixel_density(ctx) >= 0.65;
      }
      break;
    case PASS_BACK:
      if (pvr ? !pvr_units : ctx->back_mode < 1) break;
      p.family = ctx->back_mode == 5 ? FAM_CELLS : FAM_TILES;
      p.scatter_level = pvr ? 4 : std::min(4, ctx->back_mode);
      p.may_stream_table = pvr || ctx->back_mode >= 4;
// ... 212 lines not shown
  if (!strcmp(name, "coeff_lazy")) { ctx->coeff_lazy = value ? 1 : 0; return SVR_OK; }
  if (!strcmp(name, "coeff_invalidate")) { invalidate(ctx, CH_TABLE); return SVR_OK; }
  if (!strcmp(name, "coeff_table")) {
    ctx->coeff_mode = value ? 1 : 0;
    ctx->coeff_user = true;
    if (!value) invalidate(ctx, CH_TABLE_OFF);
    return SVR_OK;
  }
  if (!strcmp(name, "cell_combine")) { if (value < 0 || value > 2) return fail(ctx, SVR_E_ARG, "cell_combine: 0, 1 or 2"); ctx->cell_combine = value; return SVR_OK; }
  static const char *cwh = "cell_w / cell_h / cell_gw / cell_gh: 1..32, 0 = by the pixel density";
  static const struct { const char *n; int lo, hi; int svr_ctx::*f; const char *what; } cell_opts[] = {
      {"cell_band", 0, 10, &svr_ctx::cell_band, "cell_band: 0..10 (a run holds 2^cell_band centre planes)"},
      {"cell_qx", 1, 4, &svr_ctx::cell_qx, "cell_qx: 1, 2 or 4"},
      {"cell_w", 0, 32, &svr_ctx::cell_w, cwh}, {"cell_h", 0, 32, &svr_ctx::cell_h, cwh},
      {"cell_gw", 0, 32, &svr_ctx::cell_gw, cwh}, {"cell_gh", 0, 32, &svr_ctx::cell_gh, cwh},
      {"cell_order", 0, 20, &svr_ctx::cell_order, "cell_order: 0..20"},
      {"cell_balance", 0, 1024, &svr_ctx::cell_balance, "cell_balance: 0..1024"},
      {"cell_split", 1, 32, &svr_ctx::cell_split, "cell_split: 1..32"}};
  for (const auto &o : cell_opts) {
    if (strcmp(name, o.n)) continue;
    if (value < o.lo || value > o.hi || (o.f == &svr_ctx::cell_qx && value == 3)) return fail(ctx, SVR_E_ARG, o.what);
    ctx->*o.f = value;
    invalidate(ctx, CH_CELL_SHAPE);
    return SVR_OK;
  }
  if (!strcmp(name, "wave_groups")) { ctx->wave_groups = std::max(1, value); return SVR_OK; }
  if (!strcmp(name, "wave_cap")) { ctx->wave_cap = std::max(1024, value); ctx->wave_cap_user = true; return SVR_OK; }
  if (!strcmp(name, "reg_blind")) { ctx->reg_blind = std::max(0, value); return SVR_OK; }
  if (!strcmp(name, "reg_red_threads")) {
    if (value != 0 && value != 256 && value != 1024) return fail(ctx, SVR_E_ARG, "reg_red_threads: 0, 256 or 1024");
    ctx->reg_red_threads = value;
    return SVR_OK;
  }
  if (!strcmp(name, "reg_batch")) { ctx->reg_batch = value ? 1 : 0; return SVR_OK; }
  if (!strcmp(name, "bias_mode")) { if (value < 0 || value > 2) return fail(ctx, SVR_E_ARG, "bias_mode: 0, 1 or 2"); ctx->bias_mode = value; return SVR_OK; }
  if (!strcmp(name, "pvr_reg_levels")) { ctx->pvr_reg_levels = std::min(3, std::max(1, value)); return SVR_OK; }
  if (!strcmp(name, "pvr_reg_steps")) { ctx->pvr_reg_steps = std::max(1, value); return SVR_OK; }
  if (!strcmp(name, "pvr_reg_iterations")) { ctx->pvr_reg_iterations = std::max(1, value); return SVR_OK; }
  if (!strcmp(name, "tile_w") || !strcmp(name, "tile_h")) {
    int w = !strcmp(name, "tile_w") ? value : ctx->tile_w, h = !strcmp(name, "tile_h") ? value : ctx->tile_h;
    if (w < 1 || h < 1 || w * h > 64) return fail(ctx, SVR_E_ARG, "tile_w * tile_h must be in 1..64");
    ctx->tile_user = true;
    return set_scatter_tile(ctx, w, h);
  }
  return fail(ctx, SVR_E_ARG, std::string("unknown option ") + name);
}

int svr_get_option(svr_ctx *ctx, const char *name, int *value) {
  SVR_ENTER(ctx);
  if (!ctx || !name || !value) return SVR_E_ARG;
  int csw, csh, cgw, cgh;
  cell_sizes(ctx, csw, csh, cgw, cgh);
  const bool cells_valid = ctx->cell && ctx->cell->valid && ((cgw == csw && cgh == csh) || !ctx->cell_g || ctx->cell_g->valid);
  const struct { const char *n; int v; } tab[] = {
      {"back_mode", ctx->back_mode}, {"reg_mode", ctx->reg_mode}, {"fwd_mode", ctx->fwd_mode}, {"gauss_mode", ctx->gauss_mode}, {"pvr_mode", ctx->pvr_mode},
      {"pvr", ctx->pvr}, {"coeff_table", ctx->coeff_mode}, {"coeff_lazy", ctx->coeff_lazy}, {"coeff_valid", ctx->coeff_state != COEFF_NONE}, {"coeff_state", ctx->coeff_state}, {"tile_w", ctx->tile_w}, {"tile_h", ctx->tile_h},
      {"fwd_tile_w", ctx->fwd_tw}, {"fwd_tile_h", ctx->fwd_th}, {"wave_cap", ctx->wave_cap}, {"cell_w", csw}, {"cell_h", csh}, {"cell_gw", cgw}, {"cell_gh", cgh}, {"cell_split", ctx->cell_split}, {"cell_order", ctx->cell_order}, {"cell_balance", ctx->cell_balance}, {"cell_combine", ctx->cell_combine}, {"fwd_autotune", 0}, {"cell_qx", ctx->cell_qx}, {"fwd_unit_cap", ctx->fwd_unit_cap}, {"reg_batch", ctx->reg_batch}, {"reg_blind", ctx->reg_blind},
      {"bias_mode", ctx->bias_mode}, {"bias_corrections", ctx->bias_corrections}, {"bias_normalisations", ctx->bias_normalisations},
      {"bias_scatters", ctx->bias_scatters}, {"bias_scatters_on_cells", ctx->bias_scatters_on_cells},
      {"bias_field_bx", ctx->last_bias_bx}, {"bias_tail_lds", ctx->last_tail_lds}, {"bias_tail_rows", ctx->last_tail_rows},
      {"bias_tail_bxy", ctx->last_tail_bxy}, {"bias_tail_bxz", ctx->last_tail_bxz}, {"reg_zc", ctx->last_reg_zc}, {"reg_chunks", ctx->last_reg_chunks},
      {"psf_list_valid", ctx->psf_list_valid}, {"cells_valid", cells_valid}, {"quality_chunks", ctx->last_quality_chunks}};
  for (const auto &e : tab)
    if (!strcmp(name, e.n)) { *value = e.v; return SVR_OK; }
  return fail(ctx, SVR_E_ARG, std::string("unknown option ") + name);
}

void svr_destroy(svr_ctx *ctx) {
  if (!ctx) return;
  (void)hipSetDevice(ctx->device);
  (void)hipDeviceSynchronize();
  free_volume(ctx);
  free_slices(ctx);
  free_dev(ctx->d_mask); free_dev(ctx->d_pair_pack);
  free_dev(ctx->d_bias); free_dev(ctx->d_wb); free_dev(ctx->d_wr); free_dev(ctx->d_buffer);
  free_dev(ctx->d_bias_vol); free_dev(ctx->d_volume_weights); free_dev(ctx->d_maskC); free_dev(ctx->d_mbuf);
  free_dev(ctx->d_reg_targets);
  free_dev(ctx->d_reg_source);
  free_dev(ctx->d_pyr_full[0]); free_dev(ctx->d_pyr_full[1]); free_dev(ctx->d_pyr_a); free_dev(ctx->d_pyr_b); free_dev(ctx->d_pyr_meta);
  free_dev(ctx->d_ncc_idx); free_dev(ctx->d_ncc_m); free_dev(ctx->d_ncc_s);
  free_dev(ctx->d_nmi_io); free_dev(ctx->d_nmi_terms); free_dev(ctx->d_nmi_merge);
  free_dev(ctx->d_mot_x); free_dev(ctx->d_mot_partial); free_dev(ctx->d_mot_g);
  free_dev(ctx->d_qual_partial); free_dev(ctx->d_qual_sums);
  free_dev(ctx->d_coeff); free_dev(ctx->d_coeff_id); free_dev(ctx->d_coeff_order);
  reg_free(ctx->reg);
  cell_free(ctx->cell);
  cell_free(ctx->cell_g);
  free_dev(ctx->d_cellc);
  slab_free(ctx->slab);
  slice_em_free(ctx->sem);
  free_dev(ctx->d_spx);
  free_dev(ctx->d_counter);
  free_dev(ctx->d_out);
  free_dev(ctx->d_em_all);
  timers_resolve(ctx);
  if (ctx->ev_open) (void)hipEventDestroy(ctx->ev_open);
  for (hipEvent_t e : ctx->ev_free) (void)hipEventDestroy(e);
  ctx->ev_free.clear();
  if (ctx->own_stream && ctx->stream) (void)hipStreamDestroy(ctx->stream);
  delete ctx;
}

const char *svr_last_error(const svr_ctx *ctx) { return ctx ? ctx->err.c_str() : "null context"; }

int svr_set_flags(svr_ctx *ctx, int disable_bias_correction, int debug_gpu) {
  SVR_ENTER(ctx);
  if (!ctx) return SVR_E_ARG;
  ctx->disable_bias = disable_bias_correction != 0;
  ctx->debug_gpu = debug_gpu != 0;
  if (!ctx->disable_bias) { HIPCHK(hipSetDevice(ctx->device)); return ensure_bias_buffers(ctx); }
  return SVR_OK;
}

int svr_set_stream(svr_ctx *ctx, void *hip_stream) {
  SVR_ENTER(ctx);
  if (!ctx) return SVR_E_ARG;
  HIPCHK(hipStreamSynchronize(ctx->stream));
  if (ctx->own_stream && ctx->stream) (void)hipStreamDestroy(ctx->stream);
  ctx->stream = (hipStream_t)hip_stream;
  ctx->own_stream = false;
  return SVR_OK;
}

void *svr_get_stream(svr_ctx *ctx) { return ctx ? (void *)ctx->stream : nullptr; }
int svr_stream_sync(svr_ctx *ctx) {
  SVR_ENTER(ctx);
  if (!ctx) return SVR_E_ARG;
  HIPCHK(hipStreamSynchronize(ctx->stream));
  return SVR_OK;
}
int svr_device(svr_ctx *ctx) { return ctx ? ctx->device : -1; }
int svr_device_count(void) {
  int n = 0;
  return hipGetDeviceCount(&n) == hipSuccess ? n : 0;
}

int svr_init_reconstruction_volume(svr_ctx *ctx, const uint32_t size[3], const float dim[3],
                                   const float *data, float sigma_bias) {
  SVR_ENTER(ctx);
  if (!ctx || !size || !dim) return SVR_E_ARG;
  (void)sigma_bias;
  HIPCHK(hipSetDevice(ctx->device));
  size_t nv = (size_t)size[0] * size[1] * size[2];
  if (nv == 0 || nv >= 0xFFFFFFFFull) return fail(ctx, SVR_E_ARG, "volume size out of range");
  free_volume(ctx);
  free_dev(ctx->d_bias_vol); free_dev(ctx->d_volume_weights); free_dev(ctx->d_maskC); free_dev(ctx->d_mbuf);
  ctx->vx = size[0]; ctx->vy = size[1]; ctx->vz = size[2];
  memcpy(ctx->vdim, dim, 3 * sizeof(float));
  ctx->nv = nv;
  invalidate(ctx, CH_VOLUME_GRID);
  HIPCHK(hipMalloc(&ctx->d_recon_volw, 2 * nv * sizeof(float)));
  HIPCHK(hipMalloc(&ctx->d_addon_cmap, 2 * nv * sizeof(float)));
  HIPCHK(hipMalloc(&ctx->d_recon_new, nv * sizeof(float)));
  ctx->recon_cur = ctx->d_recon_volw;
  ctx->prep_pending = false;
  HIPCHK(hipMemsetAsync(ctx->d_recon_volw, 0, 2 * nv * sizeof(float), ctx->stream));
  HIPCHK(hipMemsetAsync(ctx->d_addon_cmap, 0, 2 * nv * sizeof(float), ctx->stream));
  if (data) HIPCHK(hipMemcpyAsync(ctx->recon(), data, nv * sizeof(float), hipMemcpyHostToDevice, ctx->stream));
  HIPCHK(hipStreamSynchronize(ctx->stream));
  return SVR_OK;
}

int svr_set_mask(svr_ctx *ctx, const uint32_t size[3], const float dim[3], const float *data,
                 float sigma_bias) {
  SVR_ENTER(ctx);
  if (!ctx || !size || !data) return SVR_E_ARG;
  (void)dim;
// ... 1226 lines not shown
  }
  HIPCHK(hipStreamSynchronize(ctx->stream));
  ctx->reg_vx = sx; ctx->reg_vy = sy; ctx->reg_vz = sz;
  return SVR_OK;
}

int svr_ncc_evaluate(svr_ctx *ctx, int n_eval, const int *target_index, const double *matrices,
                     int64_t *sums6, double *ncc) {
  SVR_ENTER(ctx);
  if (!ctx || n_eval <= 0 || !target_index || !matrices) return SVR_E_ARG;
  NEED(ctx->d_reg_targets && ctx->d_reg_source, "svr_ncc_set_targets / svr_ncc_set_source first");
  for (int i = 0; i < n_eval; ++i)
    if (target_index[i] < 0 || target_index[i] >= ctx->reg_n) return fail(ctx, SVR_E_ARG, "target index out of range");
  if ((size_t)n_eval > ctx->ncc_cap) {
    free_dev(ctx->d_ncc_idx); free_dev(ctx->d_ncc_m); free_dev(ctx->d_ncc_s);
    ctx->ncc_cap = 0;
    const size_t cap = std::max<size_t>(256, (size_t)n_eval * 3 / 2);
    HIPCHK(hipMalloc(&ctx->d_ncc_idx, cap * sizeof(int)));
    HIPCHK(hipMalloc(&ctx->d_ncc_m, cap * 16 * sizeof(double)));
    HIPCHK(hipMalloc(&ctx->d_ncc_s, cap * 6 * sizeof(long long)));
    ctx->ncc_cap = cap;
  }
  int *d_idx = ctx->d_ncc_idx;
  double *d_m = ctx->d_ncc_m;
  long long *d_s = ctx->d_ncc_s;
  std::vector<long long> h((size_t)n_eval * 6);
  hipError_t e = hipMemcpyAsync(d_idx, target_index, n_eval * sizeof(int), hipMemcpyHostToDevice, ctx->stream);
  if (e == hipSuccess) e = hipMemcpyAsync(d_m, matrices, (size_t)n_eval * 16 * sizeof(double), hipMemcpyHostToDevice, ctx->stream);
  if (e == hipSuccess) {
    hipLaunchKernelGGL(k_ncc, dim3(n_eval), dim3(256), 0, ctx->stream, ctx->d_reg_targets, ctx->reg_tx, ctx->reg_ty,
                       d_idx, d_m, ctx->d_reg_source, (int)ctx->reg_vx, (int)ctx->reg_vy, (int)ctx->reg_vz, d_s);
    e = hipGetLastError();
  }
  if (e == hipSuccess) e = hipMemcpyAsync(h.data(), d_s, h.size() * sizeof(long long), hipMemcpyDeviceToHost, ctx->stream);
  if (e == hipSuccess) e = hipStreamSynchronize(ctx->stream);
  if (e != hipSuccess) return fail(ctx, (int)e, "svr_ncc_evaluate");
  for (int i = 0; i < n_eval; ++i) {
    const long long *s = &h[6 * (size_t)i];
    if (sums6) for (int k = 0; k < 6; ++k) sums6[6 * (size_t)i + k] = s[k];
    if (ncc) {
      const double n = (double)s[0], x = (double)s[1], y = (double)s[2], x2 = (double)s[3], y2 = (double)s[4],
                   xy = (double)s[5];
      ncc[i] = n > 0 ? (xy - (x * y) / n) / (sqrt(x2 - x * x / n) * sqrt(y2 - y * y / n)) : 0.0;
    }
  }
  return SVR_OK;
}

int svr_timer_enable(svr_ctx *ctx, int enable) {
  SVR_ENTER(ctx);
  if (!ctx) return SVR_E_ARG;
  timers_resolve(ctx);
  ctx->timers = enable != 0;
  return SVR_OK;
}
int svr_timer_reset(svr_ctx *ctx) {
  SVR_ENTER(ctx);
  if (!ctx) return SVR_E_ARG;
  timers_resolve(ctx);
  for (int i = 0; i < SVR_T_COUNT; ++i) { ctx->t_ms[i] = 0; ctx->t_n[i] = 0; }
  return SVR_OK;
}
int svr_timer_get(svr_ctx *ctx, int which, double *ms_total, long *launches) {
  SVR_ENTER(ctx);
  if (!ctx || which < 0 || which >= SVR_T_COUNT) return SVR_E_ARG;
  timers_resolve(ctx);
  if (ms_total) *ms_total = ctx->t_ms[which];
  if (launches) *launches = ctx->t_n[which];
  return SVR_OK;
}
int svr_unit_counts(svr_ctx *ctx, uint64_t out3[3]) {
  SVR_ENTER(ctx);
  if (!ctx || !out3) return SVR_E_ARG;
  int r = ready(ctx);
  if (r) return r;
  if ((r = cell_prepare(ctx))) return r;
  const CellState &cs = *ctx->cell;
  const uint64_t ns = ctx->pvr ? PVR_N : PSF_SUPPORT;
  out3[0] = cs.n_sorted;
  out3[1] = (uint64_t)cs.n_sorted * ns - cs.dead_units;
  out3[2] = cs.dead_units;
  return SVR_OK;
}
int svr_cell_stats(svr_ctx *ctx, uint64_t out8[8]) {
  SVR_ENTER(ctx);
  if (!ctx || !out8) return SVR_E_ARG;
  int r = ready(ctx);
  if (r) return r;
  for (int k = 0; k < 8; ++k) out8[k] = 0;
  if ((r = cell_prepare(ctx))) return r;
  const CellState &cs = *ctx->cell;
  out8[0] = cs.a.nitems; out8[1] = cs.n_runs; out8[2] = cs.n_sorted;
  out8[3] = (uint64_t)cs.a.nents * cs.a.PP * sizeof(f2);
  CellState *g = nullptr;
  if ((r = cell_prepare_gather(ctx, g))) return r;
  if (g) { out8[4] = g->a.nitems; out8[5] = g->n_runs; out8[6] = (uint64_t)g->n_sorted * (ctx->pvr ? PVR_N : PSF_SUPPORT) * sizeof(f2); }
  out8[7] = (uint64_t)cs.a.CX << 32 | (uint64_t)cs.a.CL;
  return SVR_OK;
}
int svr_timer_begin(svr_ctx *ctx, int which) {
  SVR_ENTER(ctx);
  if (!ctx || which < 0 || which >= SVR_T_COUNT) return SVR_E_ARG;
  if (ctx->timers) {
    if (!ctx->ev_open) ctx->ev_open = timer_event(ctx);
    if (ctx->ev_open) HIPCHK(hipEventRecord(ctx->ev_open, ctx->stream));
  }
  return SVR_OK;
}
int svr_timer_end(svr_ctx *ctx, int which) {
  SVR_ENTER(ctx);
  if (!ctx || which < 0 || which >= SVR_T_COUNT) return SVR_E_ARG;
  if (ctx->timers && ctx->ev_open) {
    timer_close(ctx, which, ctx->ev_open);
    ctx->ev_open = nullptr;
  }
  return SVR_OK;
}
int svr_timer_add(svr_ctx *ctx, int which, double ms) {
  if (!ctx || which < 0 || which >= SVR_T_COUNT) return SVR_E_ARG;
  if (ctx->timers) { ctx->t_ms[which] += ms; ctx->t_n[which] += 1; }
  return SVR_OK;
}
__global__ __launch_bounds__(256) void k_clock_probe(float *out, int n) {
  f2 x[8];
#pragma unroll
  for (int k = 0; k < 8; ++k) x[k] = (f2){1.0f + 1.0e-7f * (float)(threadIdx.x + k), 1.0f - 1.0e-7f * (float)(threadIdx.x + k)};
  const f2 a = (f2){0.99999994f, 1.00000012f}, b = (f2){1.0e-9f, -1.0e-9f};
  for (int i = 0; i < n; i += 8) {
#pragma unroll
    for (int k = 0; k < 8; ++k) x[k] = fma2(x[k], a, b);
  }
  f2 t = x[0];
#pragma unroll
  for (int k = 1; k < 8; ++k) t = t + x[k];
  if (t.x == 12345.678f && t.y == 1.0f) out[blockIdx.x] = t.x;
}
int svr_clock_probe(svr_ctx *ctx, int chain, double *ms) {
  SVR_ENTER(ctx);
  if (!ctx || !ms || chain <= 0) return SVR_E_ARG;
  float *d = nullptr;
  HIPCHK(hipMalloc(&d, 4096 * sizeof(float)));
  hipEvent_t a = nullptr, b = nullptr;
  hipError_t e = hipEventCreate(&a);
  if (e == hipSuccess) e = hipEventCreate(&b);
  float best = 3.0e38f;
  for (int rep = 0; rep < 4 && e == hipSuccess; ++rep) {
    e = hipEventRecord(a, ctx->stream);
    hipLaunchKernelGGL(k_clock_probe, dim3(1024), dim3(256), 0, ctx->stream, d, chain);
    if (e == hipSuccess) e = hipEventRecord(b, ctx->stream);
    if (e == hipSuccess) e = hipEventSynchronize(b);
    float t = 0.0f;
    if (e == hipSuccess) e = hipEventElapsedTime(&t, a, b);
    if (rep > 0 && t < best) best = t;
  }
  if (a) (void)hipEventDestroy(a);
  if (b) (void)hipEventDestroy(b);
  (void)hipFree(d);
  if (e != hipSuccess) return fail(ctx, (int)e, std::string("svr_clock_probe: ") + hipGetErrorString(e));
  *ms = best;
  return SVR_OK;
}
int svr_fallbacks(svr_ctx *ctx, uint64_t out4[4]) {
  SVR_ENTER(ctx);
  if (!ctx || !out4) return SVR_E_ARG;
  for (int k = 0; k < 4; ++k) out4[k] = ctx->fallbacks[k];
  return SVR_OK;
// ... 23 lines not shown
```

fetalreconstruction_amd/csrc/svr_tile.inc:

```
struct BoxWalk {
  int x, y, z, r;
  int Px, Pxy, tx, ty, tz, tr, wx, wy;
  __device__ __forceinline__ void init(int i0, int stride, int Px_, int Pxy_) {
    Px = Px_; Pxy = Pxy_;
    z = i0 / Pxy; r = i0 - z * Pxy; y = r / Px; x = r - y * Px;
    tz = stride / Pxy; tr = stride - tz * Pxy; ty = tr / Px; tx = tr - ty * Px;
    wy = Pxy / Px; wx = Pxy - wy * Px;
  }
  __device__ __forceinline__ void step() {
    z += tz; r += tr; x += tx; y += ty;
    if (x >= Px) { x -= Px; ++y; }
    if (r >= Pxy) {
      r -= Pxy; ++z; x -= wx; y -= wy;
      if (x < 0) { x += Px; --y; }
    }
  }
};

__global__ __launch_bounds__(TILE_WAVES * 64) void back_tiled_kernel(PsfArgs a, TileArgs ta) {
  constexpr bool GAUSS1_ACT = false;
  extern __shared__ __attribute__((aligned(16))) float tile[];
  __shared__ int sh_lo[3], sh_hi[3];
  __shared__ uint32_t sh_pix[64];
  const int TILE_W = ta.tw, TILE_H = ta.th;
// ... 446 lines not shown
    for (int k = 0; k < 3; ++k) { lo[k] = __builtin_amdgcn_readfirstlane(mn[k]); hi[k] = __builtin_amdgcn_readfirstlane(mx[k]); }
  }
  __syncthreads();
  const int lox = lo[0] - NC, hix = hi[0] + NH;
  const int loy = lo[1] - NC, hiy = min(hi[1] + NH, vgy - 1);
  const int loz = lo[2] - NC, hiz = min(hi[2] + NH, vgz - 1);
  const int Dy = hiy - loy + 1, Dz = hiz - loz + 1;
  if (lox > vg.vx - 1 || Dy <= 0 || Dz <= 0) return;
  const int PL = (hix - lox + 1) | 1;
  const int PP = PL * Dy;
  if (Dz > 64 || 4 * PP > ta.cap || TILE_W * TILE_H > WAVE_MAXPIX) {
    if (lane == 0 && grp == 0) fallback_tiles[atomicAdd(fallback_count, 1u)] = t;
    return;
  }
  const RowConst RC = load_row_const(S);
  uint32_t deadbits = 0u;
  if (!PVR) {
    static_assert(PVR || NS == 16, "four pixels of 16 units per pass of the dead-unit test");
    for (int m = 0; m * 4 < npix; ++m) {
      const int k = m * 4 + (lane >> 4), z = lane & 15;
      const PixelRec R = sh_px[min(k, npix - 1)];
      const bool d = k < npix && unit_is_dead(RC, R.bx, R.by, R.bz, F, (float)(z - NC));
      const unsigned long long bd = __ballot(d);
      if ((lane >> 2) == m) deadbits = (uint32_t)(bd >> (16 * (lane & 3))) & 0xFFFFu;
    }
  }
  int nl = 0, nd = 0;
  for (int k = 0; k < npix; ++k) {
    const int czk = sh_px[k].cz;
    const uint32_t dk = (uint32_t)__shfl((int)deadbits, k, 64);
    const int z = loz + lane - czk + NC;
    if (lane < Dz && z >= 0 && z < NS) {
      if ((dk >> z) & 1u) ++nd; else ++nl;
    }
  }
  const unsigned long long mlive = __ballot(nl > 0), mdead = __ballot(nl == 0 && nd > 0);
  const int nlive = __popcll(mlive), nused = nlive + __popcll(mdead);
  if (grp * 4 >= nused) return;
  const unsigned long long below = (1ull << lane) - 1ull;
  const int pos = nl > 0 ? __popcll(mlive & below) : (nd > 0 ? nlive + __popcll(mdead & below) : -1);
  const int mycz = lane < npix ? sh_px[lane].cz : 0;
  const int slot = lane >> 4;
  const int y = lane & 15;
  const float fyl = (float)(y - NC);
  for (int j0 = grp * 4; j0 < nused; j0 += groups * 4) {
    int pl[4];
    int p = -1, mynl = 0, mynd = 0;
#pragma unroll
    for (int q = 0; q < 4; ++q) {
      const unsigned long long m = __ballot(pos == j0 + q);
      pl[q] = m ? (int)__builtin_ctzll(m) : -1;
      const int src = m ? pl[q] : 0;
      const int a_nl = __shfl(nl, src, 64), a_nd = __shfl(nd, src, 64);
      if (slot == q) { p = pl[q]; mynl = m ? a_nl : 0; mynd = m ? a_nd : 0; }
      bool isl = false, isd = false;
      if (m && lane < npix) {
        const int z = loz + pl[q] - mycz + NC;
        if (z >= 0 && z < NS) {
          isd = (deadbits >> z) & 1u;
          isl = !isd;
        }
      }
      const unsigned long long bl = __ballot(isl), bdd = __ballot(isd);
      if (isl) sh_list[q][__popcll(bl & below)] = (unsigned char)lane;
      if (isd) sh_list[q][WAVE_MAXPIX - 1 - __popcll(bdd & below)] = (unsigned char)lane;
    }
    for (int i = lane; i < 4 * PP; i += 64) box[i] = (f2){0.0f, 0.0f};
    __syncthreads();

    if (p >= 0) {
      const int P = loz + p;
      f2 *pb = box + slot * PP - lox;
      auto add_unit = [&](const PixelRec &R, const float (&out)[NS], const f2 (&acc)[NS], bool rowok, int rb) {
        if (rowok) {
          const f2 ff = (f2){R.f0, R.f1};
#pragma unroll
          for (int x = 0; x < NS; ++x) pb[rb + x] = fma2(bc2(out[x]), ff, acc[x]);
        }
      };
      if (COEFF) {
        float4 ring[3][NS / 4];
        auto request = [&](int i, float4 (&dst)[NS / 4]) {
          const int k1 = sh_list[slot][i];
          const float4 *src = a.coeff + ((size_t)sh_pid[k1] * NS + (size_t)(P - sh_px[k1].cz + NC)) * (NS / 4 * 16) + (y < NS ? y : 0);
#pragma unroll
          for (int q = 0; q < NS / 4; ++q) dst[q] = load_stream(src + q * 16);
        };
#pragma unroll
        for (int r3 = 0; r3 < 3; ++r3) if (r3 < mynl) request(r3, ring[r3]);
        for (int i0 = 0; i0 < mynl; i0 += 3) {
#pragma unroll
          for (int r3 = 0; r3 < 3; ++r3) {
            const int i = i0 + r3;
            if (i < mynl) {
              const PixelRec R = sh_px[sh_list[slot][i]];
              const int ay = R.cy + y - NC;
              const bool rowok = y < NS && ay < vgy;
              const int rb = rowok ? (ay - loy) * PL + R.cx - NC : lox;
              f2 acc[NS];
#pragma unroll
              for (int x = 0; x < NS; ++x) acc[x] = pb[rb + x];
              float out[NS];
#pragma unroll
              for (int q = 0; q < NS / 4; ++q) { out[4 * q] = ring[r3][q].x; out[4 * q + 1] = ring[r3][q].y; out[4 * q + 2] = ring[r3][q].z; out[4 * q + 3] = ring[r3][q].w; }
              if (i + 3 < mynl) request(i + 3, ring[r3]);
              add_unit(R, out, acc, rowok, rb);
            }
          }
        }
      } else {
        for (int i = 0; i < mynl; ++i) {
          const PixelRec R = sh_px[sh_list[slot][i]];
          const float fzu = (float)(P - R.cz);
          const int ay = R.cy + y - NC;
          const bool rowok = y < NS && ay < vgy;
          const int rb = rowok ? (ay - loy) * PL + R.cx - NC : lox;
          f2 acc[NS];
#pragma unroll
          for (int x = 0; x < NS; ++x) acc[x] = pb[rb + x];
          float out[NS];
          eval_row_t<NS, PVR, true>(RC, R.bx, R.by, R.bz, swap ? fzu : fyl, swap ? fyl : fzu, out);
          add_unit(R, out, acc, rowok, rb);
        }
      }
      if (!PVR) {
        for (int i = 0; i < mynd; i += 2) {
          const bool two = i + 1 < mynd;
          const PixelRec Ra = sh_px[sh_list[slot][WAVE_MAXPIX - 1 - i]];
          const PixelRec Rb = sh_px[sh_list[slot][two ? WAVE_MAXPIX - 2 - i : WAVE_MAXPIX - 1 - i]];
          const float fua = (float)(P - Ra.cz), fub = (float)(P - Rb.cz);
          const float fya = swap ? fua : fyl, fza = swap ? fyl : fua, fyb = swap ? fub : fyl, fzb = swap ? fyl : fub;
          const f2 rowx = (f2){__builtin_fmaf(RC.Lp[1], fya, __builtin_fmaf(RC.Lp[2], fza, Ra.bx)),
                               __builtin_fmaf(RC.Lp[1], fyb, __builtin_fmaf(RC.Lp[2], fzb, Rb.bx))};
          const f2 rowy = (f2){__builtin_fmaf(RC.Lp[4], fya, __builtin_fmaf(RC.Lp[5], fza, Ra.by)),
                               __builtin_fmaf(RC.Lp[4], fyb, __builtin_fmaf(RC.Lp[5], fzb, Rb.by))};
          const f2 rowz = (f2){__builtin_fmaf(RC.Lp[7], fya, __builtin_fmaf(RC.Lp[8], fza, Ra.bz)),
                               __builtin_fmaf(RC.Lp[7], fyb, __builtin_fmaf(RC.Lp[8], fzb, Rb.bz))};
          f2 xs[1], ys[1], t0[1];
          xs[0] = fma2(bc2(RC.Lp[0]), bc2((float)(-NC)), rowx);
          ys[0] = fma2(bc2(RC.Lp[3]), bc2((float)(-NC)), rowy);
          eval_pairs_xyz<1, false>(RC, xs, ys, t0);
          const f2 v = t0[0] * gauss_first_tap2<NC>(RC, rowz);
          const int aya = Ra.cy + y - NC, ayb = Rb.cy + y - NC;
          if (aya < vgy) {
            f2 *q = pb + (aya - loy) * PL + Ra.cx - NC;
            *q = fma2(bc2(v.x), (f2){Ra.f0, Ra.f1}, *q);
          }
          if (two && ayb < vgy) {
            f2 *q = pb + (ayb - loy) * PL + Rb.cx - NC;
            *q = fma2(bc2(v.y), (f2){Rb.f0, Rb.f1}, *q);
          }
        }
      }
    }
    __syncthreads();
    {
      constexpr int FLUSH_U = COEFF ? 10 : 8;
      RowWalk w0;
      w0.init(lane, 64, PL);
      asm volatile("" : "+v"(w0.x));
      if (PP <= 64 * FLUSH_U) {
        int eoff[FLUSH_U];
        {
          RowWalk w = w0;
#pragma unroll
          for (int u = 0; u < FLUSH_U; ++u) {
            const bool ok = lane + 64 * u < PP && w.x + lox < vg.vx;
            eoff[u] = ok ? (int)(sat0(w.x + lox) + sat0(w.y + loy) * sty) : -1;
            w.step();
// ... 6 lines not shown
            const f2 *pq = box + q * PP + lane;
            const float *mz = a.mask + sat0(pl[q] + loz) * stz;
            float *az_ = a.addon + sat0(pl[q] + loz) * stz, *cz_ = a.cmap + sat0(pl[q] + loz) * stz;
            f2 v[FLUSH_U];
            float mk[FLUSH_U];
#pragma unroll
            for (int u = 0; u < FLUSH_U; ++u) {
              v[u] = lane + 64 * u < PP ? pq[64 * u] : (f2){0.0f, 0.0f};
              const bool ok = eoff[u] >= 0 && (v[u].x != 0.0f || v[u].y != 0.0f);
              mk[u] = ok ? mz[eoff[u]] : 0.0f;
            }
#pragma unroll
            for (int u = 0; u < FLUSH_U; ++u) {
              if (mk[u] != 0.0f) {
                unsafeAtomicAdd(az_ + eoff[u], v[u].x);
                unsafeAtomicAdd(cz_ + eoff[u], v[u].y);
              }
            }
          }
        } else {
          float mk[4][FLUSH_U];
  #pragma unroll
          for (int q = 0; q < 4; ++q) {
            const float *mz = a.mask + sat0(max(pl[q], 0) + loz) * stz;
  #pragma unroll
            for (int u = 0; u < FLUSH_U; ++u) mk[q][u] = (pl[q] >= 0 && eoff[u] >= 0) ? mz[eoff[u]] : 0.0f;
          }
  #pragma unroll
          for (int q = 0; q < 4; ++q) {
            if (pl[q] < 0) continue;
            const f2 *pq = box + q * PP + lane;
            float *az_ = a.addon + sat0(pl[q] + loz) * stz, *cz_ = a.cmap + sat0(pl[q] + loz) * stz;
            f2 v[FLUSH_U];
  #pragma unroll
            for (int u = 0; u < FLUSH_U; ++u) v[u] = lane + 64 * u < PP ? pq[64 * u] : (f2){0.0f, 0.0f};
  #pragma unroll
            for (int u = 0; u < FLUSH_U; ++u) {
              if (mk[q][u] != 0.0f && (v[u].x != 0.0f || v[u].y != 0.0f)) {
                unsafeAtomicAdd(az_ + eoff[u], v[u].x);
                unsafeAtomicAdd(cz_ + eoff[u], v[u].y);
              }
            }
          }
        }
      } else {
        for (int q = 0; q < 4; ++q) {
          if (pl[q] < 0) continue;
          RowWalk w = w0;
          const f2 *pq = box + q * PP;
          const uint32_t zoff = sat0(pl[q] + loz) * stz;
          for (int i = lane; i < PP; i += 64, w.step()) {
            const f2 v = pq[i];
            if ((v.x != 0.0f || v.y != 0.0f) && w.x + lox < vg.vx) {
              const uint32_t vi = sat0(w.x + lox) + sat0(w.y + loy) * sty + zoff;
              if (a.mask[vi] != 0.0f) {
                unsafeAtomicAdd(a.addon + vi, v.x);
                unsafeAtomicAdd(a.cmap + vi, v.y);
              }
            }
          }
        }
      }
    }
    if (j0 + groups * 4 < nused) __syncthreads();
  }
}


#ifndef FWDU_WAVES
#define FWDU_WAVES 8
#endif
#define FWDU_MAXPIX 32
template <bool GAUSS1, int NS = PSF_SUPPORT, bool PVR = false, bool COEFF = false>
__global__ __launch_bounds__(FWDU_WAVES * 64) void fwd_unit_kernel(PsfArgs a, TileArgs ta) {
  constexpr int NC = (NS - 1) / 2, NH = NS - 1 - NC;
  constexpr int US = 16;
  constexpr int T = FWDU_WAVES * 64;
  extern __shared__ __attribute__((aligned(16))) float tile[];
  f2 *box = reinterpret_cast<f2 *>(tile);
  __shared__ int sh_lo[3], sh_hi[3];
  __shared__ PixelRec sh_px[FWDU_MAXPIX];
  __shared__ uint32_t sh_idx[FWDU_MAXPIX];
  __shared__ uint32_t sh_pid[COEFF ? FWDU_MAXPIX : 1];
  __shared__ uint32_t sh_dead[FWDU_MAXPIX];
  __shared__ unsigned short sh_units[FWDU_MAXPIX * US];
  __shared__ f2 sh_part[FWDU_MAXPIX * US];
  __shared__ double sh_partd[GAUSS1 ? FWDU_MAXPIX * US : 1];
  __shared__ uint32_t sh_hit[FWDU_MAXPIX];
  __shared__ int sh_npix, sh_nlive, sh_ndead;
  const int TILE_W = ta.tw, TILE_H = ta.th;
  const int wave = __builtin_amdgcn_readfirstlane(threadIdx.x >> 6);
  const int lane = threadIdx.x & 63;
  const VolGeom &vg = a.vg;
  const uint32_t t = ta.tiles[xcd_run_index(blockIdx.x, ta.ntiles)];
  const int per_slice = ta.tiles_x * ta.tiles_y;
  const uint32_t sl = t / per_slice;
  const int r = t - sl * per_slice;
  const int ty = r / ta.tiles_x, tx = r - ty * ta.tiles_x;
  const SliceConst &S = a.sc[sl];
  const uint32_t n2 = (uint32_t)(a.sx * a.sy);
  const bool swap = S.own == 1;
  const int F = swap ? 1 : 2;

  if (threadIdx.x < 3) { sh_lo[threadIdx.x] = INT_MAX; sh_hi[threadIdx.x] = INT_MIN; }
  if (threadIdx.x < FWDU_MAXPIX) { sh_dead[threadIdx.x] = 0u; sh_hit[threadIdx.x] = 0u; }
  if (threadIdx.x == 0) { sh_nlive = 0; sh_ndead = 0; }
  __syncthreads();
  if (wave == 0) {
    const int px = tx * TILE_W + (lane % TILE_W), py = ty * TILE_H + (lane / TILE_W);
    bool act = false;
    uint32_t idx = 0;
    if (lane < TILE_W * TILE_H && px < a.sx && py < a.sy) {
      idx = (uint32_t)px + (uint32_t)py * a.sx + sl * n2;
      act = pixel_active(a.slices, GAUSS1 ? (const float *)nullptr : a.psf_sums, a.flag, idx);
    }
    unsigned long long b = __ballot(act);
    if (act) {
      PixelState P = pixel_setup(S, vg, px, py);
      PixelRec R;
      R.cx = P.cxi; R.cy = P.cyi; R.cz = P.czi; R.bx = P.bx; R.by = P.by; R.bz = P.bz;
      R.f1 = GAUSS1 ? 0.0f : 1.0f / a.psf_sums[idx]; R.f0 = 0.0f;
      const int k = __popcll(b & ((1ull << lane) - 1ull));
      sh_px[k] = R;
      sh_idx[k] = idx;
      if (COEFF) sh_pid[k] = a.coeff_id[idx];
      atomicMin(&sh_lo[0], P.cxi); atomicMax(&sh_hi[0], P.cxi);
      atomicMin(&sh_lo[1], P.cyi); atomicMax(&sh_hi[1], P.cyi);
      atomicMin(&sh_lo[2], P.czi); atomicMax(&sh_hi[2], P.czi);
    }
    if (lane == 0) sh_npix = __popcll(b);
  }
  __syncthreads();
  const int npix = sh_npix;
  const int lox = sh_lo[0] - NC, hix = sh_hi[0] + NH;
  const int loy = sh_lo[1] - NC, hiy = min(sh_hi[1] + NH, vg.vy - 1);
  const int loz = sh_lo[2] - NC, hiz = min(sh_hi[2] + NH, vg.vz - 1);
  const int Dx = hix - lox + 1, Dy = hiy - loy + 1, Dz = hiz - loz + 1;
  if (lox > vg.vx - 1 || Dy <= 0 || Dz <= 0) return;
  const int Px = Dx | 1;
  const int Pxy = Px * Dy + ((Px * Dy) & 1 ? 0 : 1);
  const bool in_lds = (long long)Pxy * Dz <= (long long)ta.cap;
  const uint32_t sxy = (uint32_t)(vg.vx * vg.vy);
  const RowConst RC = load_row_const(S);
  if (in_lds) {
    const int vox = Pxy * Dz;
    BoxWalk bw;
    bw.init(threadIdx.x, T, Px, Pxy);
    for (int i = threadIdx.x; i < vox; i += T, bw.step()) {
      const int gx = bw.x + lox;
      f2 v = (f2){0.0f, 0.0f};
      if (bw.y < Dy && bw.x < Dx && gx < vg.vx) {
        const uint32_t vi = sat0(gx) + sat0(bw.y + loy) * (uint32_t)vg.vx + sat0(bw.z + loz) * sxy;
        if (!GAUSS1 && a.volm) {
          const float2 t = a.volm[vi];
          v = (f2){t.x, t.y};
        } else {
          const float vraw = (GAUSS1 || PVR) ? 0.0f : a.vol[vi];
          const float m = a.mask[vi] != 0.0f ? 1.0f : 0.0f;
          v = GAUSS1 ? (f2){1.0f, m}
                     : (f2){m != 0.0f ? (PVR ? pvr_tex(a.vol, vg, (int)sat0(gx), (int)sat0(bw.y + loy), (int)sat0(bw.z + loz)) : vraw) : 0.0f, m};
        }
      }
      box[i] = v;
    }
  }
  {
    static_assert(FWDU_MAXPIX * 16 <= T, "one unit per thread");
    __shared__ int sh_wlive[FWDU_WAVES];
    const int i = threadIdx.x;
    const int k = i / NS, u = i % NS;
    bool live = false;
    if (i < npix * NS) {
      const PixelRec R = sh_px[k];
      const int cu = swap ? R.cy : R.cz;
      const bool inb = cu + u - NC < (swap ? vg.vy : vg.vz);
      if (inb) {
        const bool dead = !PVR && unit_is_dead(RC, R.bx, R.by, R.bz, F, (float)(u - NC));
        if (dead) {
          atomicOr(&sh_dead[k], 1u << u);
          sh_units[FWDU_MAXPIX * US - 1 - atomicAdd(&sh_ndead, 1)] = (unsigned short)(k << 4 | u);
        } else {
          live = true;
        }
      } else {
        sh_part[k * US + u] = (f2){0.0f, 0.0f};
        if (GAUSS1) sh_partd[k * US + u] = 0.0;
      }
    }
    const unsigned long long bl = __ballot(live);
    if (lane == 0) sh_wlive[wave] = __popcll(bl);
    __syncthreads();
    int base = 0, tot = 0;
#pragma unroll
    for (int w = 0; w < FWDU_WAVES; ++w) { const int c = sh_wlive[w]; base += w < wave ? c : 0; tot += c; }
    if (live) sh_units[base + __popcll(bl & ((1ull << lane) - 1ull))] = (unsigned short)(k << 4 | u);
    if (threadIdx.x == 0) sh_nlive = tot;
  }
  __syncthreads();
  const int nlive = sh_nlive, ndead = sh_ndead;
  const int slot = lane >> 4, y = lane & 15;
  const float fyl = (float)(y - NC);
  auto live_unit = [&](const int j0) {
    const int j = j0 + slot;
    const bool valid = j < nlive;
    const int ku = sh_units[valid ? j : j0];
    const int k = ku >> 4, u = ku & 15;
    const PixelRec R = sh_px[k];
    const float fu = (float)(u - NC);
    const int ay = R.cy + (swap ? u : y) - NC, az = R.cz + (swap ? y : u) - NC;
    const bool rowok = valid && y < NS && ay < vg.vy && az < vg.vz;
    float out[NS];
    if (COEFF) {
      const float4 *src = a.coeff + ((size_t)sh_pid[k] * NS + (size_t)u) * (NS / 4 * 16) + (y < NS ? y : 0);
#pragma unroll
      for (int q = 0; q < NS / 4; ++q) {
        const float4 c = load_stream(src + q * 16);
        out[4 * q] = c.x; out[4 * q + 1] = c.y; out[4 * q + 2] = c.z; out[4 * q + 3] = c.w;
      }
    } else {
      eval_row_t<NS, PVR, true>(RC, R.bx, R.by, R.bz, swap ? fu : fyl, swap ? fyl : fu, out);
    }
    f2 acc = (f2){0.0f, 0.0f};
    double accd = 0.0;
    bool hit = false;
    if (in_lds) {
      const f2 *pb = box + (rowok ? (ay - loy) * Px + (az - loz) * Pxy + R.cx - NC - lox : 0);
      f2 v[NS];
#pragma unroll
      for (int x = 0; x < NS; ++x) v[x] = pb[x];
#pragma unroll
      for (int x = 0; x < NS; ++x) {
        if (GAUSS1) {
          accd += (double)(out[x] * v[x].x);
          hit = hit | ((v[x].y != 0.0f) & (__float_as_uint(out[x]) != 0x80000000u));
        } else {
          acc = fma2(bc2(out[x]), v[x], acc);
        }
      }
    } else {
      for (int x = 0; x < NS; ++x) {
        const int gx = R.cx + x - NC;
        f2 v = (f2){0.0f, 0.0f};
        if (rowok && gx < vg.vx) {
          const uint32_t vi = sat0(gx) + sat0(ay) * (uint32_t)vg.vx + sat0(az) * sxy;
          const float m = a.mask[vi] != 0.0f ? 1.0f : 0.0f;
          v = GAUSS1 ? (f2){1.0f, m} : (f2){m != 0.0f ? (PVR ? pvr_tex(a.vol, vg, (int)sat0(gx), (int)sat0(ay), (int)sat0(az)) : a.vol[vi]) : 0.0f, m};
        }
        if (GAUSS1) {
          accd += (double)(out[x] * v.x);
          hit = hit | ((v.y != 0.0f) & (__float_as_uint(out[x]) != 0x80000000u));
        } else {
          acc = fma2(bc2(out[x]), v, acc);
        }
      }
    }
    if (!rowok) { acc = (f2){0.0f, 0.0f}; accd = 0.0; hit = false; }
    if (GAUSS1) accd = row_sum16(accd);
    else { acc.x = row_sum16(acc.x); acc.y = row_sum16(acc.y); }
    if (GAUSS1) {
      const bool anyhit = ((uint32_t)(__ballot(hit) >> (16 * slot)) & 0xFFFFu) != 0u;
      if (valid && y == 0) {
        sh_partd[k * US + u] = accd;
        if (anyhit) atomicOr(&sh_hit[k], 1u << u);
      }
    } else if (valid && y == 0) {
      sh_part[k * US + u] = acc;
    }
  };
  for (int j0 = wave * 4; j0 < nlive; j0 += FWDU_WAVES * 4) live_unit(j0);
  for (int j0 = wave * 8; !PVR && j0 < ndead; j0 += FWDU_WAVES * 8) {
    const int ja = j0 + 2 * slot, jb = ja + 1;
    const bool va = ja < ndead, vb = jb < ndead;
    const int kua = sh_units[FWDU_MAXPIX * US - 1 - (va ? ja : j0)], kub = sh_units[FWDU_MAXPIX * US - 1 - (vb ? jb : j0)];
    const PixelRec Ra = sh_px[kua >> 4], Rb = sh_px[kub >> 4];
    const float fua = (float)((kua & 15) - NC), fub = (float)((kub & 15) - NC);
    const float fya = swap ? fua : fyl, fza = swap ? fyl : fua, fyb = swap ? fub : fyl, fzb = swap ? fyl : fub;
    const f2 rowx = (f2){__builtin_fmaf(RC.Lp[1], fya, __builtin_fmaf(RC.Lp[2], fza, Ra.bx)),
                         __builtin_fmaf(RC.Lp[1], fyb, __builtin_fmaf(RC.Lp[2], fzb, Rb.bx))};
    const f2 rowy = (f2){__builtin_fmaf(RC.Lp[4], fya, __builtin_fmaf(RC.Lp[5], fza, Ra.by)),
                         __builtin_fmaf(RC.Lp[4], fyb, __builtin_fmaf(RC.Lp[5], fzb, Rb.by))};
    const f2 rowz = (f2){__builtin_fmaf(RC.Lp[7], fya, __builtin_fmaf(RC.Lp[8], fza, Ra.bz)),
                         __builtin_fmaf(RC.Lp[7], fyb, __builtin_fmaf(RC.Lp[8], fzb, Rb.bz))};
    f2 xs[1], ys[1], t0[1];
    xs[0] = fma2(bc2(RC.Lp[0]), bc2((float)(-NC)), rowx);
    ys[0] = fma2(bc2(RC.Lp[3]), bc2((float)(-NC)), rowy);
    eval_pairs_xyz<1, false>(RC, xs, ys, t0);
    const f2 v = t0[0] * gauss_first_tap2<PSF_CENTRE>(RC, rowz);
    f2 wa = (f2){0.0f, 0.0f}, wb = (f2){0.0f, 0.0f};
    {
      const int aya = Ra.cy + (int)fya, aza = Ra.cz + (int)fza, ayb = Rb.cy + (int)fyb, azb = Rb.cz + (int)fzb;
      if (in_lds) {
        if (va && aya < vg.vy && aza < vg.vz) wa = box[(aya - loy) * Px + (aza - loz) * Pxy + Ra.cx - NC - lox];
        if (vb && ayb < vg.vy && azb < vg.vz) wb = box[(ayb - loy) * Px + (azb - loz) * Pxy + Rb.cx - NC - lox];
      } else {
        if (va && aya < vg.vy && aza < vg.vz && Ra.cx - NC < vg.vx) {
          const uint32_t vi = sat0(Ra.cx - NC) + sat0(aya) * (uint32_t)vg.vx + sat0(aza) * sxy;
          const float m = a.mask[vi] != 0.0f ? 1.0f : 0.0f;
          wa = GAUSS1 ? (f2){1.0f, m} : (f2){m != 0.0f ? a.vol[vi] : 0.0f, m};
        }
// ... 63 lines not shown
```

fetalreconstruction_amd/engine.py:

```python
from __future__ import annotations

import ctypes as C
import os

import numpy as np

_HERE = os.path.dirname(os.path.abspath(__file__))
LIB_PATH = os.environ.get("SVR_HIP_LIB") or os.path.join(_HERE, "lib", "libsvr_hip.so")

BUF_RECONSTRUCTED, BUF_VOL_WEIGHTS, BUF_ADDON, BUF_CONFIDENCE_MAP, BUF_MASK = 0, 1, 2, 3, 4
BUF_BIAS_VOLUME, BUF_SMOOTH_MASK = 5, 6
BUF_SLICES, BUF_WEIGHTS, BUF_SIMSLICES, BUF_SIMWEIGHTS, BUF_PSF_SUMS, BUF_BIAS = 10, 11, 12, 13, 14, 15
BUF_SIMINSIDE, BUF_VOXEL_COUNT = 20, 21
T_BACKPROJECT, T_FORWARD, T_GAUSS, T_REGULARIZE, T_ESTEP, T_MSTEP, T_SCALE, T_REGISTER = range(8)
TIMER_NAMES = ("backproject", "forward", "gauss", "regularize", "estep", "mstep", "scale", "register", "allreduce", "exchange_host", "coeff_build", "reduce_scatter", "allgather",
               "backproject_table", "forward_table", "forward_store", "backproject_store")

EXPORTS = [
    "svr_create", "svr_destroy", "svr_last_error", "svr_set_flags", "svr_set_option", "svr_get_option", "svr_set_spx_masks", "svr_init_reconstruction_volume",
    "svr_set_mask", "svr_init_storage_volumes", "svr_fill_slices", "svr_set_slice_dims",
    "svr_set_slice_matrices", "svr_generate_psf_volume", "svr_update_scale_vector",
    "svr_update_slice_weights", "svr_update_reconstructed", "svr_sync_cpu", "svr_get_vol_weights",
    "svr_gaussian_reconstruction", "svr_simulate_slices", "svr_initialize_em_values",
    "svr_initialize_robust_statistics", "svr_estep", "svr_mstep", "svr_calculate_scale_vector",
    "svr_superresolution", "svr_mask_volume", "svr_scale_volume", "svr_restore_slice_intensities",
    "svr_debug_get", "svr_debug_set", "svr_debug_probe_pixel", "svr_device_ptr", "svr_volume_voxels", "svr_set_stream",
    "svr_gaussian_reconstruction_local", "svr_gaussian_reconstruction_finish",
    "svr_superresolution_backproject", "svr_superresolution_update", "svr_robust_statistics_sums",
    "svr_mstep_sums", "svr_scale_volume_sums", "svr_scale_volume_apply", "svr_timer_get",
    "svr_unit_counts", "svr_fallbacks", "svr_clock_probe", "svr_slice_em_setup", "svr_slice_em_set_state", "svr_mstep_estep_device", "svr_slice_em_run", "svr_slice_em_apply_weights", "svr_slice_em_fetch", "svr_slice_em_set_patch_form", "svr_cell_stats", "svr_pair_pack", "svr_pair_unpack", "svr_timer_reset", "svr_timer_enable", "svr_timer_begin", "svr_timer_end", "svr_timer_add", "svr_counters", "svr_get_stream", "svr_device", "svr_device_count", "svr_combine_weights", "svr_update_stack_sizes", "svr_ncc_set_targets", "svr_ncc_set_source",
    "svr_ncc_evaluate", "svr_ncc_alloc_targets", "svr_pyr_upload", "svr_pyr_level", "svr_nmi_bin_source", "svr_nmi_evaluate", "svr_stack_motion", "svr_slice_quality", "svr_correct_bias", "svr_normalise_bias", "svr_normalise_bias_local",
    "svr_normalise_bias_finish", "svr_init_reg_storage_volumes", "svr_fill_reg_slices",
    "svr_update_resampled_slices_i2w", "svr_prepare_slice_to_volume_reg", "svr_register_slices_to_volume",
    "svr_reg_set_schedule", "svr_reg_evaluate_costs", "svr_reg_counters", "svr_pvr_cc_patches", "svr_pvr_register_patches",
    "svr_slab_plan", "svr_slab_rs_pack", "svr_slab_update", "svr_slab_finish", "svr_stream_sync",
    "svr_get_scale_vector", "svr_adopt_scale_vector", "svr_get_slice_inside", "svr_mstep_estep", "svr_mstep_sums_fetch", "svr_mstep_partial", "svr_mstep_estep_ranks",
]


class SvrError(RuntimeError):
    pass


_lib = None


def load_library(path: str = LIB_PATH):
    global _lib
    if _lib is None:
        if not os.path.exists(path):
            raise SvrError(f"{path} not found: build the HIP engine first (fetalreconstruction_amd/build.py); "
                           "there is no CPU fallback")
        lib = C.CDLL(path)
        lib.svr_last_error.restype = C.c_char_p
        lib.svr_device_ptr.restype = C.c_void_p
        lib.svr_volume_voxels.restype = C.c_size_t
        lib.svr_destroy.restype = None
        _lib = lib
    return _lib


def _p(a):
    return a.ctypes.data_as(C.c_void_p)


def _f32(a):
    return np.ascontiguousarray(a, dtype=np.float32)


def _u3(v):
    return (C.c_uint32 * 3)(*[int(x) for x in v])


def _f3(v):
    return (C.c_float * 3)(*[float(x) for x in v])


class Reconstruction:

    def __init__(self, device: int = 0):
        self._lib = load_library()
        h = C.c_void_p()
        rc = self._lib.svr_create(int(device), C.byref(h))
        if rc != 0 or not h:
            raise SvrError(f"svr_create(device={device}) failed with status {rc} (no usable MI355X / HIP device?)")
        self._h = h
        self.vsize = None
        self.sgrid = None

    def close(self):
        if getattr(self, "_h", None):
            self._lib.svr_destroy(self._h)
            self._h = None

    def __del__(self):
        try:
            self.close()
        except Exception:
            pass

    def _ck(self, rc):
        if rc != 0:
            msg = self._lib.svr_last_error(self._h)
            raise SvrError(f"status {rc}: {msg.decode() if msg else ''}")

    def InitReconstructionVolume(self, size, dim, data=None, sigma_bias=12.0):
        d = _f32(data) if data is not None else None
        self._ck(self._lib.svr_init_reconstruction_volume(self._h, _u3(size), _f3(dim), _p(d) if d is not None else None,
                                                          C.c_float(sigma_bias)))
        self.vsize = tuple(int(s) for s in size)

    def setMask(self, size, dim, data, sigma_bias=12.0):
        d = _f32(data)
# ... 287 lines not shown

    def registerSlicesToVolume(self, transf):
        t = _f32(transf).reshape(-1).copy()
        if t.size != 16 * self._reg_grid[0]:
            raise SvrError("registerSlicesToVolume: one Matrix4 per slice expected")
        self._ck(self._lib.svr_register_slices_to_volume(self._h, _p(t)))
        return t.reshape(-1, 4, 4)

    def evaluate_costs(self, transf, level, active=None):
        ns, H, W = self._reg_grid
        t = _f32(transf).reshape(-1)
        act = None if active is None else np.ascontiguousarray(active, np.int32)
        a = ns if act is None else len(act)
        sim = np.zeros(ns, np.float32)
        dbg = np.zeros((3, a, H, W), np.float32)
        self._ck(self._lib.svr_reg_evaluate_costs(self._h, _p(t), int(level), None if act is None else _p(act), a,
                                                  _p(sim), _p(dbg)))
        return sim, dbg

    def cc_patches(self, ri2w, tmats, level, buffers=None):
        n = self.sgrid[0]
        r, t = _f32(ri2w).reshape(n, 16), _f32(tmats).reshape(n, 16)
        b = None if buffers is None else _f32(buffers)
        out = np.zeros(n, np.float32)
        sums = np.zeros((n, 6), np.float64)
        self._ck(self._lib.svr_pvr_cc_patches(self._h, None if b is None else _p(b), _p(r), _p(t), int(level), _p(out),
                                              _p(sums)))
        return out, sums

    def register_patches(self, ri2w, mo, invmo, transformations):
        n = self.sgrid[0]
        r, m, mi = (_f32(a).reshape(n, 16) for a in (ri2w, mo, invmo))
        t = _f32(transformations).reshape(n, 16).copy()
        ti = np.zeros((n, 16), np.float32)
        c = np.zeros(3, np.int64)
        self._ck(self._lib.svr_pvr_register_patches(self._h, _p(r), _p(m), _p(mi), _p(t), _p(ti), _p(c)))
        return t, ti, c

    def reg_counters(self):
        c = np.zeros(4, np.int64)
        self._ck(self._lib.svr_reg_counters(self._h, _p(c)))
        return c

    def set_spx_masks(self, masks):
        if masks is None:
            self._ck(self._lib.svr_set_spx_masks(self._h, None))
        else:
            m = np.ascontiguousarray(masks, np.uint8)
            self._ck(self._lib.svr_set_spx_masks(self._h, _p(m)))

    def set_option(self, name, value):
        self._ck(self._lib.svr_set_option(self._h, name.encode(), int(value)))

    def get_option(self, name):
        v = C.c_int(0)
        self._ck(self._lib.svr_get_option(self._h, name.encode(), C.byref(v)))
        return v.value

    def probe_pixel(self, sl, px, py):
        v = np.zeros(4096, np.float32)
        c = np.zeros(3, np.int32)
        self._ck(self._lib.svr_debug_probe_pixel(self._h, int(sl), int(px), int(py), _p(v), _p(c)))
        return v, c

    def timer_enable(self, on=True):
        self._ck(self._lib.svr_timer_enable(self._h, int(bool(on))))

    def timer_reset(self):
        self._ck(self._lib.svr_timer_reset(self._h))

    def timers(self):
        out = {}
        for i, name in enumerate(TIMER_NAMES):
            ms, n = C.c_double(0), C.c_long(0)
            self._ck(self._lib.svr_timer_get(self._h, i, C.byref(ms), C.byref(n)))
            out[name] = (ms.value, n.value)
        return out

    def unit_counts(self):
        o = (C.c_uint64 * 3)()
        self._ck(self._lib.svr_unit_counts(self._h, o))
        return dict(pixels=int(o[0]), live_units=int(o[1]), dead_units=int(o[2]))

    def slab_chunks(self, world, rank):
        a, b = C.c_size_t(0), C.c_size_t(0)
        self._ck(self._lib.svr_slab_plan(self._h, int(world), int(rank), C.byref(a), C.byref(b)))
        return int(a.value), int(b.value)

    def cell_stats(self):
        o = (C.c_uint64 * 8)()
        self._ck(self._lib.svr_cell_stats(self._h, o))
        return dict(items=int(o[0]), runs=int(o[1]), sorted_pixels=int(o[2]), staging_bytes=int(o[3]), gather_items=int(o[4]),
                    gather_runs=int(o[5]), gather_partial_bytes=int(o[6]), cell=(int(o[7]) >> 32, int(o[7]) & 0xFFFFFFFF))

    def fallbacks(self):
        o = (C.c_uint64 * 4)()
        self._ck(self._lib.svr_fallbacks(self._h, o))
        return dict(scatter_to_atomics=int(o[0]), gather_to_tiles=int(o[1]), gauss1_to_tiles=int(o[2]), tiles_rerun=int(o[3]))

    def clock_probe(self, chain=1 << 20):
        ms = C.c_double()
        self._ck(self._lib.svr_clock_probe(self._h, int(chain), C.byref(ms)))
        return ms.value, int(chain)

    def counters(self):
        o = (C.c_uint64 * 8)()
        self._ck(self._lib.svr_counters(self._h, o))
        return dict(Vs=int(o[0]), active=int(o[1]), Va=int(o[2]), Nv=int(o[3]), slices=int(o[4]),
                    tiles=int(o[5]), fallback_tiles=int(o[6]), rerun8_tiles=int(o[7]))


def device_count():
    return int(load_library().svr_device_count())


def sync_gpu(rec: Reconstruction, prob, quality_factor: float = 2.0):
    from . import geometry as geo

    vs, vd = prob.vsize, prob.vdim
    rec.InitReconstructionVolume(vs, vd, None, 12.0)
    rec.setMask(vs, vd, prob.mask, 12.0)
    ns, sy, sx = prob.slices.shape
    rec.initStorageVolumes((sx, sy, ns), tuple(prob.slice_dim[0]))
    rec.FillSlices(prob.slices, prob.sizes_x, prob.sizes_y)
    rec.setSliceDims(prob.slice_dim, quality_factor)
    a = geo.ImageAttributes(128, 128, 128, *[float(d) for d in vd])
    rec.generatePSFVolume(None, (128, 128, 128), tuple(prob.slice_dim[0]), vd,
                          geo.to_matrix4(geo.image_to_world(a)), geo.to_matrix4(geo.world_to_image(a)),
                          quality_factor)
    rec.SetSliceMatrices(prob.slice_t, prob.slice_tinv, prob.slice_i2w, prob.slice_w2i, prob.slice_i2w,
                         prob.slice_w2i, prob.recon_i2w, prob.recon_w2i)
```

include/svr_hip.h:

```cpp
#ifndef SVR_HIP_H
#define SVR_HIP_H

#include <stddef.h>
#include <stdint.h>

#ifdef __cplusplus
extern "C" {
#endif

typedef struct svr_ctx svr_ctx;

#define SVR_OK 0
#define SVR_E_ARG 10001
#define SVR_E_STATE 10002

int svr_create(int device, svr_ctx **out);
void svr_destroy(svr_ctx *ctx);
const char *svr_last_error(const svr_ctx *ctx);
int svr_set_flags(svr_ctx *ctx, int disable_bias_correction, int debug_gpu);
int svr_set_option(svr_ctx *ctx, const char *name, int value);
int svr_get_option(svr_ctx *ctx, const char *name, int *value);
int svr_set_spx_masks(svr_ctx *ctx, const char *masks_or_null);

int svr_init_reconstruction_volume(svr_ctx *ctx, const uint32_t size[3], const float dim[3],
// ... 62 lines not shown
int svr_debug_set(svr_ctx *ctx, int which, const void *host_in, size_t bytes);
int svr_debug_probe_pixel(svr_ctx *ctx, int slice, int px, int py, float *vals4096, int *centre3);

void *svr_device_ptr(svr_ctx *ctx, int which);
int svr_pair_pack(svr_ctx *ctx, int which, size_t n_floats, void **packed, size_t *n_packed);
int svr_pair_unpack(svr_ctx *ctx, int which, size_t n_floats);
size_t svr_volume_voxels(const svr_ctx *ctx);
int svr_set_stream(svr_ctx *ctx, void *hip_stream);
void *svr_get_stream(svr_ctx *ctx);
int svr_stream_sync(svr_ctx *ctx);
int svr_device(svr_ctx *ctx);
int svr_device_count(void);
int svr_gaussian_reconstruction_local(svr_ctx *ctx);
int svr_gaussian_reconstruction_finish(svr_ctx *ctx, int *voxel_num_local);
int svr_superresolution_backproject(svr_ctx *ctx, const float *slice_weight);
int svr_superresolution_update(svr_ctx *ctx, int adaptive, float alpha, float min_intensity,
                               float max_intensity, float delta, float lambda);
int svr_slab_plan(svr_ctx *ctx, int world, int rank, size_t *rs_floats_per_rank, size_t *ag_floats_per_rank);
int svr_slab_rs_pack(svr_ctx *ctx, void **send, void **recv);
int svr_slab_update(svr_ctx *ctx, int adaptive, float alpha, float min_intensity, float max_intensity, float delta, float lambda,
                    void **send, void **recv);
int svr_slab_finish(svr_ctx *ctx);
int svr_normalise_bias_local(svr_ctx *ctx);
int svr_normalise_bias_finish(svr_ctx *ctx, float sigma_bias);
int svr_robust_statistics_sums(svr_ctx *ctx, double out2[2]);
int svr_mstep_sums(svr_ctx *ctx, double out5[5]);
int svr_scale_volume_sums(svr_ctx *ctx, double out2[2]);
int svr_scale_volume_apply(svr_ctx *ctx, float scale);

int svr_ncc_set_targets(svr_ctx *ctx, int n, int tx, int ty, const int16_t *targets);
typedef struct svr_pyr_image {
  double i2w_out[12];
  double w2i_in[12];
  int pad;
} svr_pyr_image;
int svr_ncc_alloc_targets(svr_ctx *ctx, int n, int tx, int ty);
int svr_pyr_upload(svr_ctx *ctx, int slot, const int16_t *images, size_t count);
int svr_pyr_level(svr_ctx *ctx, int slot, size_t offset, int n_images, const int in_dims[3], const double *kernel_x, int size_x,
                  const double *kernel_y, int size_y, const double *kernel_z, int size_z, int resample, const int out_dims[3],
                  const svr_pyr_image *images, int first_plane, int *min_out, int *max_out);
int svr_ncc_set_source(svr_ctx *ctx, const uint32_t size[3], const int16_t *source_or_null);
int svr_ncc_evaluate(svr_ctx *ctx, int n_eval, const int *target_index, const double *matrices,
                     int64_t *sums6_or_null, double *ncc_or_null);
int svr_nmi_bin_source(svr_ctx *ctx, int width);
int svr_nmi_evaluate(svr_ctx *ctx, int n_eval, const int *planes_per_eval, const int *target_index, const double *matrices,
                     const int *target_width, const int *target_nbins, int source_nbins, double *out4, uint32_t *hist_or_null);
int svr_stack_motion(svr_ctx *ctx, const float *slices, int m, int n, double *singular_values_or_null, double *et, int *r_min,
                     double *score);
#define SVR_SLICE_QUALITY_SUMS 10
int svr_slice_quality(svr_ctx *ctx, double *sums );

int svr_init_reg_storage_volumes(svr_ctx *ctx, const uint32_t size[3], const float dim[3]);
int svr_fill_reg_slices(svr_ctx *ctx, const float *sdata, const float *slices_resampledI2W_or_null);
int svr_update_resampled_slices_i2w(svr_ctx *ctx, const float *ofsSlice);
int svr_prepare_slice_to_volume_reg(svr_ctx *ctx);
int svr_register_slices_to_volume(svr_ctx *ctx, float *transf);
int svr_reg_set_schedule(svr_ctx *ctx, int levels, int steps, int iterations);
int svr_reg_evaluate_costs(svr_ctx *ctx, const float *transf, int level, const int *active_or_null, int n_active,
                           float *similarities_out, float *reg_slices_out_or_null);
int svr_reg_counters(svr_ctx *ctx, long long out4[4]);

int svr_pvr_cc_patches(svr_ctx *ctx, const float *buffer_or_null, const float *RI2W, const float *Tmats, int level,
                       float *ncc_out, double *sums6_or_null);
int svr_pvr_register_patches(svr_ctx *ctx, const float *RI2W, const float *Mo, const float *InvMo, float *T, float *Tinv_out,
                             long long *counters3_or_null);

enum svr_timer {
  SVR_T_BACKPROJECT = 0, SVR_T_FORWARD = 1, SVR_T_GAUSS = 2, SVR_T_REGULARIZE = 3,
  SVR_T_ESTEP = 4, SVR_T_MSTEP = 5, SVR_T_SCALE = 6, SVR_T_REGISTER = 7,
  SVR_T_ALLREDUCE = 8, SVR_T_EXCHANGE = 9,
  SVR_T_COEFF_BUILD = 10,
  SVR_T_REDUCE_SCATTER = 11, SVR_T_ALLGATHER = 12,
  SVR_T_BACKPROJECT_TABLE = 13, SVR_T_FORWARD_TABLE = 14, SVR_T_FORWARD_STORE = 15, SVR_T_BACKPROJECT_STORE = 16,
  SVR_T_COUNT = 17
};
int svr_timer_begin(svr_ctx *ctx, int which);
int svr_timer_end(svr_ctx *ctx, int which);
int svr_timer_add(svr_ctx *ctx, int which, double ms);
int svr_timer_get(svr_ctx *ctx, int which, double *ms_total, long *launches);
int svr_timer_reset(svr_ctx *ctx);
int svr_timer_enable(svr_ctx *ctx, int enable);
int svr_counters(svr_ctx *ctx, uint64_t out8[8]);
int svr_unit_counts(svr_ctx *ctx, uint64_t out3[3]);
int svr_slice_em_setup(svr_ctx *ctx, int ns_global, int world, int rank, const int *rank_lo, const int *order_or_null, double step);
int svr_slice_em_set_state(svr_ctx *ctx, const float *slice_weights_global, const unsigned char *excluded_global, const double scalars5[5],
                           const float em3[3]);
int svr_mstep_estep_device(svr_ctx *ctx, int iter, float step, void **send, void **recv, size_t *n_floats_per_rank);
int svr_slice_em_run(svr_ctx *ctx);
int svr_slice_em_apply_weights(svr_ctx *ctx);
int svr_slice_em_fetch(svr_ctx *ctx, float *scale_global, float *slice_weight_global, float *slice_potential_global,
                       unsigned char *slice_inside_global, double scalars5[5], float em3[3]);
int svr_slice_em_set_patch_form(svr_ctx *ctx, const int *source_ref_or_null);
int svr_fallbacks(svr_ctx *ctx, uint64_t out4[4]);
int svr_clock_probe(svr_ctx *ctx, int chain, double *ms);
int svr_cell_stats(svr_ctx *ctx, uint64_t out8[8]);

#ifdef __cplusplus
}
#endif
#endif
```

Before: 219.4.

## Pack PSF coefficient table units by dropping all-zero quads via keep bitmasks

Each 16x16 PSF coefficient unit now stores only its non-zero float4 quads contiguously, with a 64-bit keep mask per unit. Readers rebuild the address from a popcount rank, and dropped quads are served from a shared zero quad. This is meant to cut coefficient table reads and writes in the forward and backprojection cell and tile kernels. In exchange it adds per-unit mask loads, shuffles and popcount address arithmetic, an extra memset of the mask array per build, scattered rather than strided access, and an added lgkmcnt wait in the LDS staging path.

```diff
diff --git a/fetalreconstruction_amd/csrc/svr_cell.inc b/fetalreconstruction_amd/csrc/svr_cell.inc
--- a/fetalreconstruction_amd/csrc/svr_cell.inc
+++ b/fetalreconstruction_amd/csrc/svr_cell.inc
@@ -490,6 +490,12 @@
           if (lane == 0) { atomicAdd(ca.stats + 1, 1ull); atomicAdd(ca.stats + 2, (unsigned long long)mx); }
         }
         const int w0a = (int)((unsigned short)r0.cx | ((unsigned)(unsigned short)r0.cl << 16));
+        constexpr bool PACKED = COEFF == 1 && CoeffPacked<NS, PVR>::value;
+        uint32_t klo0 = 0u, khi0 = 0u;
+        if (PACKED && act0 && !dead0) {
+          const unsigned long long km = a.coeff_keep[(size_t)(uint32_t)pid0 * NS + (size_t)(P - r0.cz + NC)];
+          klo0 = (uint32_t)km; khi0 = (uint32_t)(km >> 32);
+        }
         struct Unit { int cx, cy, cz; float bx, by, bz, f0, f1; int pid; };
         auto fetch = [&](int j) -> Unit {
           const int src = slot * SL + (j & 15);
@@ -517,7 +523,15 @@
               const int j = valid ? __builtin_ctz(ml) : 0;
               ml &= ml - 1u;
               u = fetch(j);
-              if (valid) {
+              if (PACKED) {
+                const int ks = slot * SL + (j & 15);
+                const uint32_t klo = (uint32_t)__shfl((int)klo0, ks, 64), khi = (uint32_t)__shfl((int)khi0, ks, 64);
+                if (valid) {
+                  const float4 *unit = a.coeff + ((size_t)(uint32_t)u.pid * NS + (size_t)(P - u.cz + NC)) * (NS / 4 * 16);
+#pragma unroll
+                  for (int q = 0; q < NS / 4; ++q) dst[q] = load_stream(packed_quad(unit, a.coeff_zero, klo, khi, q, y));
+                }
+              } else if (valid) {
                 const float4 *src = a.coeff + ((size_t)(uint32_t)u.pid * NS + (size_t)(P - u.cz + NC)) * (NS / 4 * 16) + (y < NS ? y : 0);
 #pragma unroll
                 for (int q = 0; q < NS / 4; ++q) dst[q] = load_stream(src + q * 16);
@@ -577,8 +591,11 @@
               float out[NS];
               eval_row_t<NS, PVR, true, SVR_CELL_EVAL_H(NS)>(RC, u.bx, u.by, u.bz, swap ? fzu : fyl, swap ? fyl : fzu, out);
               if (COEFF == 3) {
-                if (valid && y < NS) {
-                  float4 *dstp = const_cast<float4 *>(a.coeff) + ((size_t)(uint32_t)u.pid * NS + (size_t)(P - u.cz + NC)) * (NS / 4 * 16) + y;
+                const size_t un = (size_t)(uint32_t)u.pid * NS + (size_t)(P - u.cz + NC);
+                if constexpr (CoeffPacked<NS, PVR>::value) {
+                  store_unit_packed(const_cast<float4 *>(a.coeff) + un * (NS / 4 * 16), const_cast<unsigned long long *>(a.coeff_keep) + un, out, valid, slot, y);
+                } else if (valid && y < NS) {
+                  float4 *dstp = const_cast<float4 *>(a.coeff) + un * (NS / 4 * 16) + y;
 #pragma unroll
                   for (int q = 0; q < NS / 4; ++q) store_stream(dstp + q * 16, out[4 * q], out[4 * q + 1], out[4 * q + 2], out[4 * q + 3]);
                 }
@@ -942,6 +959,11 @@
         unsigned md = idle ? 0u : (unsigned)(__ballot(dead0) >> sh) & ((1u << SL) - 1u);
         const int w0a = (int)((unsigned short)r0.cx | ((unsigned)(unsigned short)r0.cl << 16));
         const uint32_t myrec = rstart + c0 + (uint32_t)mine;
+        uint32_t klo0 = 0u, khi0 = 0u;
+        if (COEFF == 2 && act0 && !dead0) {
+          const unsigned long long km = a.coeff_keep[(size_t)(uint32_t)pid0 * NS + (size_t)(P - r0.cz + NC)];
+          klo0 = (uint32_t)km; khi0 = (uint32_t)(km >> 32);
+        }
         struct Unit { int cx, cy, cz; float bx, by, bz; uint32_t rec; int pid; };
         auto fetch = [&](int j) -> Unit {
           const int src = slot * SL + (j & 15);
@@ -966,10 +988,13 @@
             mli &= mli - 1u;
             const int src = slot * SL + (j & 15);
             const int pid = __shfl(pid0, src, 64), czk = __shfl((int)r0.cz, src, 64);
-            const float4 *srcp = vi ? a.coeff + ((size_t)(uint32_t)pid * NS + (size_t)(P - czk + NC)) * (HQ * 16) + y : a.coeff + lane;
+            const uint32_t kls = (uint32_t)__shfl((int)klo0, src, 64), khs = (uint32_t)__shfl((int)khi0, src, 64);
+            const uint32_t klo = vi ? kls : 0u, khi = vi ? khs : 0u;
+            const float4 *unit = a.coeff + ((size_t)(uint32_t)pid * NS + (size_t)(P - czk + NC)) * (HQ * 16);
             const uint32_t dst = stage_lds + (uint32_t)s_issue * (HQ * 1024u);
-#pragma unroll
-            for (int q = 0; q < HQ; ++q) glds16(srcp + q * 16, dst + q * 1024u);
+            asm volatile("s_waitcnt lgkmcnt(0)" ::: "memory");
+#pragma unroll
+            for (int q = 0; q < HQ; ++q) glds16(packed_quad(unit, a.coeff_zero, klo, khi, q, y), dst + q * 1024u);
             s_issue = s_issue + 1 == DD ? 0 : s_issue + 1;
             return true;
           };
@@ -1009,6 +1034,7 @@
             if (valid && y == 0) part[(size_t)(P - u.cz + NC) * npart + u.rec] = acc;
           }
         } else if (COEFF == 1) {
+          static_assert(COEFF != 1 || !CoeffPacked<NS, PVR>::value, "support 16 reads its packed units through the LDS (COEFF == 2)");
           constexpr int RING = SVR_CELL_RING;
           float4 ring[RING][NS / 4];
           Unit ru[RING];
@@ -1071,8 +1097,11 @@
           float out[NS];
           eval_row_t<NS, PVR, true, SVR_CELL_EVAL_H_FWD(NS)>(RC, u.bx, u.by, u.bz, swap ? fzu : fyl, swap ? fyl : fzu, out);
           if (COEFF == 3) {
-            if (valid && y < NS) {
-              float4 *dstp = const_cast<float4 *>(a.coeff) + ((size_t)(uint32_t)u.pid * NS + (size_t)(P - u.cz + NC)) * (NS / 4 * 16) + y;
+            const size_t un = (size_t)(uint32_t)u.pid * NS + (size_t)(P - u.cz + NC);
+            if constexpr (CoeffPacked<NS, PVR>::value) {
+              store_unit_packed(const_cast<float4 *>(a.coeff) + un * (NS / 4 * 16), const_cast<unsigned long long *>(a.coeff_keep) + un, out, valid, slot, y);
+            } else if (valid && y < NS) {
+              float4 *dstp = const_cast<float4 *>(a.coeff) + un * (NS / 4 * 16) + y;
 #pragma unroll
               for (int q = 0; q < NS / 4; ++q) store_stream(dstp + q * 16, out[4 * q], out[4 * q + 1], out[4 * q + 2], out[4 * q + 3]);
             }
diff --git a/fetalreconstruction_amd/csrc/svr_hip.hip b/fetalreconstruction_amd/csrc/svr_hip.hip
--- a/fetalreconstruction_amd/csrc/svr_hip.hip
+++ b/fetalreconstruction_amd/csrc/svr_hip.hip
@@ -124,6 +124,8 @@
   float *addon, *cmap;
   const float4 *coeff;
   const uint32_t *coeff_id;
+  const unsigned long long *coeff_keep;
+  const float4 *coeff_zero;
 };
 
 struct PixelState {
@@ -672,8 +674,37 @@
   *p = make_float4(a, b, c, d);
 #endif
 }
+template <int NS, bool PVR> struct CoeffPacked { static constexpr bool value = NS == 16 && !PVR; };
+__device__ __forceinline__ const float4 *packed_quad(const float4 *unit, const float4 *zero, uint32_t klo, uint32_t khi, int q, int y) {
+  const int b = (q & 1) * 16 + y;
+  const uint32_t w = q < 2 ? klo : khi;
+  uint32_t rank = (uint32_t)__popc(w & ((1u << b) - 1u));
+  if (q >= 2) rank += (uint32_t)__popc(klo);
+  return (w >> b) & 1u ? unit + rank : zero;
+}
+__device__ __forceinline__ void store_unit_packed(float4 *unit, unsigned long long *keepw, const float (&out)[16], bool valid, int slot, int y) {
+  uint32_t m[4];
+#pragma unroll
+  for (int q = 0; q < 4; ++q) {
+    const bool k = (__float_as_uint(out[4 * q]) != 0x80000000u) | (__float_as_uint(out[4 * q + 1]) != 0x80000000u) |
+                   (__float_as_uint(out[4 * q + 2]) != 0x80000000u) | (__float_as_uint(out[4 * q + 3]) != 0x80000000u);
+    m[q] = (uint32_t)(__ballot(valid && k) >> (16 * slot)) & 0xFFFFu;
+  }
+  const uint32_t klo = m[0] | m[1] << 16, khi = m[2] | m[3] << 16;
+  if (valid) {
+#pragma unroll
+    for (int q = 0; q < 4; ++q) {
+      const int b = (q & 1) * 16 + y;
+      const uint32_t w = q < 2 ? klo : khi;
+      uint32_t rank = (uint32_t)__popc(w & ((1u << b) - 1u));
+      if (q >= 2) rank += (uint32_t)__popc(klo);
+      if ((w >> b) & 1u) store_stream(unit + rank, out[4 * q], out[4 * q + 1], out[4 * q + 2], out[4 * q + 3]);
+    }
+    if (y == 0) *keepw = (unsigned long long)klo | (unsigned long long)khi << 32;
+  }
+}
 template <int NS, bool PVR>
-__global__ __launch_bounds__(256) void k_coeff_build(PsfArgs a, float4 *coeff, uint32_t *coeff_id, uint32_t base) {
+__global__ __launch_bounds__(256) void k_coeff_build(PsfArgs a, float4 *coeff, uint32_t *coeff_id, unsigned long long *keep, uint32_t base) {
   constexpr int NC = (NS - 1) / 2, QUADS = NS / 4;
   static_assert(NS % 4 == 0 && NS <= 16, "tap quads, one row per lane of a 16-lane slot");
   const uint32_t wl = blockIdx.x * 4u + (threadIdx.x >> 6);
@@ -699,7 +730,9 @@
     if (__all(dead)) continue;
     float out[NS];
     eval_row_t<NS, PVR, true>(RC, P.bx, P.by, P.bz, swap ? fu : fyl, swap ? fyl : fu, out);
-    if (!dead && u < NS && y < NS) {
+    if constexpr (CoeffPacked<NS, PVR>::value) {
+      store_unit_packed(coeff + ((size_t)w * NS + u) * (QUADS * 16), keep + (size_t)w * NS + u, out, !dead, slot, y);
+    } else if (!dead && u < NS && y < NS) {
       float4 *dst = coeff + ((size_t)w * NS + u) * (QUADS * 16) + y;
 #pragma unroll
       for (int q = 0; q < QUADS; ++q) store_stream(dst + q * 16, out[4 * q], out[4 * q + 1], out[4 * q + 2], out[4 * q + 3]);
@@ -1004,6 +1037,7 @@
   bool fwd_mode_user = false;
   bool sr_no_wait = false;
   float4 *d_coeff = nullptr;
+  unsigned long long *d_coeff_keep = nullptr;
   uint32_t *d_coeff_id = nullptr;
   uint32_t *d_coeff_order = nullptr;
   size_t coeff_order_cap = 0;
@@ -1363,7 +1397,11 @@
   return a;
 }
 
-void give_coeff(const svr_ctx *ctx, PsfArgs &a) { a.coeff = ctx->d_coeff; a.coeff_id = ctx->d_coeff_id; }
+void give_coeff(const svr_ctx *ctx, PsfArgs &a) {
+  a.coeff = ctx->d_coeff; a.coeff_id = ctx->d_coeff_id;
+  a.coeff_keep = ctx->d_coeff_keep;
+  a.coeff_zero = ctx->d_coeff_keep ? reinterpret_cast<const float4 *>(ctx->d_coeff_keep + ctx->coeff_cap * PSF_SUPPORT) : nullptr;
+}
 
 int ensure_bias_buffers(svr_ctx *ctx) {
   if (ctx->disable_bias) return SVR_OK;
@@ -1448,7 +1486,7 @@
 int coeff_prepare(svr_ctx *ctx, const uint32_t **list) {
   const size_t npx = ctx->n_active;
   if (npx > ctx->coeff_cap) {
-    free_dev(ctx->d_coeff);
+    free_dev(ctx->d_coeff); free_dev(ctx->d_coeff_keep);
     ctx->coeff_cap = 0;
     size_t fr = 0, tot = 0;
     const size_t per_px = ctx->pvr ? (size_t)PVR_N * (PVR_N / 4) * 16 : (size_t)PSF_SUPPORT * (PSF_SUPPORT / 4) * 16;
@@ -1456,13 +1494,17 @@
     const char *cap_gb = getenv("SVR_COEFF_MAX_GB");
     const bool over = cap_gb && (double)bytes > atof(cap_gb) * 1073741824.0;
     const size_t bias_later = ctx->disable_bias ? 0 : (ctx->d_bias ? 0 : 4 * ctx->np * sizeof(float)) + (ctx->d_bias_vol ? 0 : 4 * ctx->nv * sizeof(float));
-    if (over || hipMemGetInfo(&fr, &tot) != hipSuccess || bytes + bias_later + (size_t(2) << 30) > fr || hipMalloc(&ctx->d_coeff, bytes) != hipSuccess) {
+    const size_t keep_bytes = ctx->pvr ? 0 : npx * PSF_SUPPORT * sizeof(unsigned long long) + sizeof(float4);
+    if (over || hipMemGetInfo(&fr, &tot) != hipSuccess || bytes + keep_bytes + bias_later + (size_t(2) << 30) > fr || hipMalloc(&ctx->d_coeff, bytes) != hipSuccess ||
+        (keep_bytes && hipMalloc(&ctx->d_coeff_keep, keep_bytes) != hipSuccess)) {
       (void)hipGetLastError();
+      free_dev(ctx->d_coeff);
       ctx->d_coeff = nullptr;
       ctx->coeff_mode = 0;
       return SVR_OK;
     }
     ctx->coeff_cap = npx;
+    if (keep_bytes) HIPCHK(hipMemsetD32Async((hipDeviceptr_t)(ctx->d_coeff_keep + npx * PSF_SUPPORT), (int)0x80000000u, 4, ctx->stream));
   }
   if (!ctx->d_coeff_id) HIPCHK(hipMalloc(&ctx->d_coeff_id, ctx->np * sizeof(uint32_t)));
   if (ctx->coeff_ids_valid && ctx->coeff_list) { *list = ctx->coeff_list; return SVR_OK; }
@@ -1472,6 +1514,10 @@
     if (r) return r;
   }
   ctx->coeff_list = *list;
+  return SVR_OK;
+}
+int coeff_keep_clear(svr_ctx *ctx) {
+  if (ctx->d_coeff_keep) HIPCHK(hipMemsetAsync(ctx->d_coeff_keep, 0, ctx->coeff_cap * PSF_SUPPORT * sizeof(unsigned long long), ctx->stream));
   return SVR_OK;
 }
 int ensure_coeff(svr_ctx *ctx) {
@@ -1483,10 +1529,11 @@
   { const int r = coeff_prepare(ctx, &a.list); if (r) return r; }
   if (!ctx->coeff_mode) return SVR_OK;
   ScopedTimer tb(ctx, SVR_T_COEFF_BUILD);
+  { const int r = coeff_keep_clear(ctx); if (r) return r; }
   {
     const int rr = pixel_list_in_pieces(a, [&](const PsfArgs &ap, uint32_t off) {
-      if (ctx->pvr) hipLaunchKernelGGL((k_coeff_build<PVR_N, true>), dim3(nblk(ap.n, 4)), dim3(256), 0, ctx->stream, ap, ctx->d_coeff, ctx->d_coeff_id, off);
-      else hipLaunchKernelGGL((k_coeff_build<PSF_SUPPORT, false>), dim3(nblk(ap.n, 4)), dim3(256), 0, ctx->stream, ap, ctx->d_coeff, ctx->d_coeff_id, off);
+      if (ctx->pvr) hipLaunchKernelGGL((k_coeff_build<PVR_N, true>), dim3(nblk(ap.n, 4)), dim3(256), 0, ctx->stream, ap, ctx->d_coeff, ctx->d_coeff_id, ctx->d_coeff_keep, off);
+      else hipLaunchKernelGGL((k_coeff_build<PSF_SUPPORT, false>), dim3(nblk(ap.n, 4)), dim3(256), 0, ctx->stream, ap, ctx->d_coeff, ctx->d_coeff_id, ctx->d_coeff_keep, off);
       KCHK("k_coeff_build");
       return (int)SVR_OK;
     });
@@ -1511,6 +1558,7 @@
     invalidate(ctx, CH_TABLE_IDS);
     ctx->coeff_ids_valid = true;
   }
+  if ((r = coeff_keep_clear(ctx))) return r;
   *store = true;
   return SVR_OK;
 }
@@ -1615,7 +1663,7 @@
   if (ch & (CH_SLICE_PIXELS | CH_PSF_SUMS | CH_TILE_SHAPE)) ctx->psf_list_valid = false;
   if (ch & (CH_TAPS | CH_SLICE_PIXELS | CH_VOLUME_GRID | CH_TABLE | CH_TABLE_OFF)) ctx->coeff_state = COEFF_NONE;
   if ((ch & CH_PSF_SUMS) && ctx->coeff_state == COEFF_PSF) ctx->coeff_state = COEFF_NONE;
-  if (ch & CH_TABLE_OFF) { free_dev(ctx->d_coeff); ctx->coeff_cap = 0; }
+  if (ch & CH_TABLE_OFF) { free_dev(ctx->d_coeff); free_dev(ctx->d_coeff_keep); ctx->coeff_cap = 0; }
   const bool cells = ch & (CH_TAPS | CH_SLICE_PIXELS | CH_VOLUME_GRID | CH_CELL_SHAPE | CH_TABLE_OFF);
   if (cells) ctx->cellc_valid = ctx->coeff_ids_valid = false;
   for (CellState *cs : {ctx->cell, ctx->cell_g}) {
@@ -1994,7 +2042,7 @@
   free_dev(ctx->d_nmi_io); free_dev(ctx->d_nmi_terms); free_dev(ctx->d_nmi_merge);
   free_dev(ctx->d_mot_x); free_dev(ctx->d_mot_partial); free_dev(ctx->d_mot_g);
   free_dev(ctx->d_qual_partial); free_dev(ctx->d_qual_sums);
-  free_dev(ctx->d_coeff); free_dev(ctx->d_coeff_id); free_dev(ctx->d_coeff_order);
+  free_dev(ctx->d_coeff); free_dev(ctx->d_coeff_keep); free_dev(ctx->d_coeff_id); free_dev(ctx->d_coeff_order);
   reg_free(ctx->reg);
   cell_free(ctx->cell);
   cell_free(ctx->cell_g);
@@ -3387,6 +3435,85 @@
   out3[2] = cs.dead_units;
   return SVR_OK;
 }
+__global__ void k_coeff_census(const unsigned long long *keep, size_t n, unsigned long long *out2) {
+  unsigned long long q = 0, u = 0;
+  for (size_t i = (size_t)blockIdx.x * blockDim.x + threadIdx.x; i < n; i += (size_t)gridDim.x * blockDim.x) {
+    const unsigned long long m = keep[i];
+    q += (unsigned long long)__popcll(m); u += m != 0ull;
+  }
+  for (int o = 32; o; o >>= 1) { q += __shfl_xor(q, o, 64); u += __shfl_xor(u, o, 64); }
+  if ((threadIdx.x & 63) == 0) { atomicAdd(out2, q); atomicAdd(out2 + 1, u); }
+}
+__global__ __launch_bounds__(64) void k_coeff_unpack(const float4 *coeff, const unsigned long long *keep, const float4 *zero, const uint32_t *pids,
+                                                      uint32_t cap, int plane0, int nplanes, float4 *dense, unsigned long long *keep_out) {
+  const uint32_t i = blockIdx.x;
+  const uint32_t pid = pids[i / (uint32_t)nplanes];
+  const size_t un = (size_t)pid * PSF_SUPPORT + (size_t)(plane0 + (int)(i % (uint32_t)nplanes));
+  const unsigned long long m = pid < cap ? keep[un] : 0ull;
+  const int b = threadIdx.x;
+  if (dense) dense[(size_t)i * 64 + b] = *packed_quad(coeff + un * 64, zero, (uint32_t)m, (uint32_t)(m >> 32), b >> 4, b & 15);
+  if (keep_out && b == 0) keep_out[i] = m;
+}
+__global__ void k_coeff_pids(const uint32_t *coeff_id, const uint32_t *idx, uint32_t n, uint32_t *pid) {
+  const uint32_t i = blockIdx.x * blockDim.x + threadIdx.x;
+  if (i < n) pid[i] = coeff_id[idx[i]];
+}
+static bool packed_table_there(const svr_ctx *ctx) { return ctx->coeff_mode && ctx->coeff_state != COEFF_NONE && ctx->d_coeff && ctx->d_coeff_keep && ctx->d_coeff_id; }
+int svr_coeff_kept_quads(svr_ctx *ctx, uint64_t out3[3]) {
+  SVR_ENTER(ctx);
+  if (!ctx || !out3) return SVR_E_ARG;
+  out3[0] = out3[1] = out3[2] = 0;
+  if (!packed_table_there(ctx)) return SVR_OK;
+  const size_t n = (size_t)ctx->n_active * PSF_SUPPORT;
+  unsigned long long *d = nullptr, h[2] = {0, 0};
+  HIPCHK(hipMalloc(&d, sizeof(h)));
+  hipError_t e = hipMemsetAsync(d, 0, sizeof(h), ctx->stream);
+  if (e == hipSuccess) {
+    hipLaunchKernelGGL(k_coeff_census, dim3((unsigned)std::min<size_t>((n + 255) / 256, 4096)), dim3(256), 0, ctx->stream, ctx->d_coeff_keep, n, d);
+    e = hipMemcpyAsync(h, d, sizeof(h), hipMemcpyDeviceToHost, ctx->stream);
+  }
+  if (e == hipSuccess) e = hipStreamSynchronize(ctx->stream);
+  (void)hipFree(d);
+  HIPCHK(e);
+  out3[0] = h[0]; out3[1] = h[1]; out3[2] = n;
+  return SVR_OK;
+}
+static int coeff_unpack(svr_ctx *ctx, const uint32_t *idx, const uint32_t *pid_in, uint32_t n, int plane0, int nplanes, uint32_t *pid, uint64_t *keep, float *dense) {
+  if (!packed_table_there(ctx)) return SVR_E_ARG;
+  const size_t nu = (size_t)n * nplanes;
+  uint32_t *d_idx = nullptr, *d_pid = nullptr;
+  unsigned long long *d_keep = nullptr;
+  float4 *d_dense = nullptr;
+  hipError_t e = hipMalloc(&d_idx, n * sizeof(uint32_t));
+  if (e == hipSuccess) e = hipMalloc(&d_pid, n * sizeof(uint32_t));
+  if (e == hipSuccess) e = hipMalloc(&d_keep, nu * sizeof(unsigned long long));
+  if (e == hipSuccess && dense) e = hipMalloc(&d_dense, nu * 64 * sizeof(float4));
+  if (e == hipSuccess) e = hipMemcpyAsync(idx ? d_idx : d_pid, idx ? idx : pid_in, n * sizeof(uint32_t), hipMemcpyHostToDevice, ctx->stream);
+  if (e == hipSuccess) {
+    if (idx) hipLaunchKernelGGL(k_coeff_pids, dim3(nblk(n)), dim3(256), 0, ctx->stream, ctx->d_coeff_id, d_idx, n, d_pid);
+    const float4 *zero = reinterpret_cast<const float4 *>(ctx->d_coeff_keep + ctx->coeff_cap * PSF_SUPPORT);
+    hipLaunchKernelGGL(k_coeff_unpack, dim3((unsigned)nu), dim3(64), 0, ctx->stream, ctx->d_coeff, ctx->d_coeff_keep, zero, d_pid, (uint32_t)ctx->coeff_cap, plane0, nplanes, d_dense, d_keep);
+    e = hipGetLastError();
+  }
+  if (e == hipSuccess && pid) e = hipMemcpyAsync(pid, d_pid, n * sizeof(uint32_t), hipMemcpyDeviceToHost, ctx->stream);
+  if (e == hipSuccess && keep) e = hipMemcpyAsync(keep, d_keep, nu * sizeof(unsigned long long), hipMemcpyDeviceToHost, ctx->stream);
+  if (e == hipSuccess && dense) e = hipMemcpyAsync(dense, d_dense, nu * 64 * sizeof(float4), hipMemcpyDeviceToHost, ctx->stream);
+  if (e == hipSuccess) e = hipStreamSynchronize(ctx->stream);
+  (void)hipFree(d_idx); (void)hipFree(d_pid); (void)hipFree(d_keep); (void)hipFree(d_dense);
+  HIPCHK(e);
+  return SVR_OK;
+}
+int svr_coeff_read_pixels(svr_ctx *ctx, const uint32_t *idx, uint32_t n, uint32_t *pid, uint64_t *keep, float *dense) {
+  SVR_ENTER(ctx);
+  if (!ctx || !idx || !n || n > (1u << 20)) return SVR_E_ARG;
+  for (uint32_t i = 0; i < n; ++i) if (idx[i] >= ctx->np) return SVR_E_ARG;
+  return coeff_unpack(ctx, idx, nullptr, n, 0, PSF_SUPPORT, pid, keep, dense);
+}
+int svr_coeff_read_unit(svr_ctx *ctx, uint32_t pid, int plane, float out[256]) {
+  SVR_ENTER(ctx);
+  if (!ctx || !out || plane < 0 || plane >= PSF_SUPPORT || pid >= ctx->n_active) return SVR_E_ARG;
+  return coeff_unpack(ctx, nullptr, &pid, 1, plane, 1, nullptr, nullptr, out);
+}
 int svr_cell_stats(svr_ctx *ctx, uint64_t out8[8]) {
   SVR_ENTER(ctx);
   if (!ctx || !out8) return SVR_E_ARG;
diff --git a/fetalreconstruction_amd/csrc/svr_tile.inc b/fetalreconstruction_amd/csrc/svr_tile.inc
--- a/fetalreconstruction_amd/csrc/svr_tile.inc
+++ b/fetalreconstruction_amd/csrc/svr_tile.inc
@@ -552,9 +552,16 @@
         float4 ring[3][NS / 4];
         auto request = [&](int i, float4 (&dst)[NS / 4]) {
           const int k1 = sh_list[slot][i];
-          const float4 *src = a.coeff + ((size_t)sh_pid[k1] * NS + (size_t)(P - sh_px[k1].cz + NC)) * (NS / 4 * 16) + (y < NS ? y : 0);
-#pragma unroll
-          for (int q = 0; q < NS / 4; ++q) dst[q] = load_stream(src + q * 16);
+          const size_t un = (size_t)sh_pid[k1] * NS + (size_t)(P - sh_px[k1].cz + NC);
+          if constexpr (CoeffPacked<NS, PVR>::value) {
+            const unsigned long long km = a.coeff_keep[un];
+#pragma unroll
+            for (int q = 0; q < NS / 4; ++q) dst[q] = load_stream(packed_quad(a.coeff + un * (NS / 4 * 16), a.coeff_zero, (uint32_t)km, (uint32_t)(km >> 32), q, y));
+          } else {
+            const float4 *src = a.coeff + un * (NS / 4 * 16) + (y < NS ? y : 0);
+#pragma unroll
+            for (int q = 0; q < NS / 4; ++q) dst[q] = load_stream(src + q * 16);
+          }
         };
 #pragma unroll
         for (int r3 = 0; r3 < 3; ++r3) if (r3 < mynl) request(r3, ring[r3]);
@@ -727,6 +734,8 @@
   __shared__ PixelRec sh_px[FWDU_MAXPIX];
   __shared__ uint32_t sh_idx[FWDU_MAXPIX];
   __shared__ uint32_t sh_pid[COEFF ? FWDU_MAXPIX : 1];
+  constexpr bool PACKED = COEFF && CoeffPacked<NS, PVR>::value;
+  __shared__ unsigned long long sh_keep[PACKED ? FWDU_MAXPIX * 16 : 1];
   __shared__ uint32_t sh_dead[FWDU_MAXPIX];
   __shared__ unsigned short sh_units[FWDU_MAXPIX * US];
   __shared__ f2 sh_part[FWDU_MAXPIX * US];
@@ -826,6 +835,7 @@
           sh_units[FWDU_MAXPIX * US - 1 - atomicAdd(&sh_ndead, 1)] = (unsigned short)(k << 4 | u);
         } else {
           live = true;
+          if (PACKED) sh_keep[k * US + u] = a.coeff_keep[(size_t)sh_pid[k] * NS + (size_t)u];
         }
       } else {
         sh_part[k * US + u] = (f2){0.0f, 0.0f};
@@ -856,10 +866,11 @@
     const bool rowok = valid && y < NS && ay < vg.vy && az < vg.vz;
     float out[NS];
     if (COEFF) {
-      const float4 *src = a.coeff + ((size_t)sh_pid[k] * NS + (size_t)u) * (NS / 4 * 16) + (y < NS ? y : 0);
+      const float4 *unit = a.coeff + ((size_t)sh_pid[k] * NS + (size_t)u) * (NS / 4 * 16);
+      const unsigned long long km = PACKED ? sh_keep[k * US + u] : 0ull;
 #pragma unroll
       for (int q = 0; q < NS / 4; ++q) {
-        const float4 c = load_stream(src + q * 16);
+        const float4 c = load_stream(PACKED ? packed_quad(unit, a.coeff_zero, (uint32_t)km, (uint32_t)(km >> 32), q, y) : unit + q * 16 + (y < NS ? y : 0));
         out[4 * q] = c.x; out[4 * q + 1] = c.y; out[4 * q + 2] = c.z; out[4 * q + 3] = c.w;
       }
     } else {
diff --git a/fetalreconstruction_amd/engine.py b/fetalreconstruction_amd/engine.py
--- a/fetalreconstruction_amd/engine.py
+++ b/fetalreconstruction_amd/engine.py
@@ -28,7 +28,7 @@
     "svr_gaussian_reconstruction_local", "svr_gaussian_reconstruction_finish",
     "svr_superresolution_backproject", "svr_superresolution_update", "svr_robust_statistics_sums",
     "svr_mstep_sums", "svr_scale_volume_sums", "svr_scale_volume_apply", "svr_timer_get",
-    "svr_unit_counts", "svr_fallbacks", "svr_clock_probe", "svr_slice_em_setup", "svr_slice_em_set_state", "svr_mstep_estep_device", "svr_slice_em_run", "svr_slice_em_apply_weights", "svr_slice_em_fetch", "svr_slice_em_set_patch_form", "svr_cell_stats", "svr_pair_pack", "svr_pair_unpack", "svr_timer_reset", "svr_timer_enable", "svr_timer_begin", "svr_timer_end", "svr_timer_add", "svr_counters", "svr_get_stream", "svr_device", "svr_device_count", "svr_combine_weights", "svr_update_stack_sizes", "svr_ncc_set_targets", "svr_ncc_set_source",
+    "svr_unit_counts", "svr_coeff_kept_quads", "svr_coeff_read_unit", "svr_coeff_read_pixels", "svr_fallbacks", "svr_clock_probe", "svr_slice_em_setup", "svr_slice_em_set_state", "svr_mstep_estep_device", "svr_slice_em_run", "svr_slice_em_apply_weights", "svr_slice_em_fetch", "svr_slice_em_set_patch_form", "svr_cell_stats", "svr_pair_pack", "svr_pair_unpack", "svr_timer_reset", "svr_timer_enable", "svr_timer_begin", "svr_timer_end", "svr_timer_add", "svr_counters", "svr_get_stream", "svr_device", "svr_device_count", "svr_combine_weights", "svr_update_stack_sizes", "svr_ncc_set_targets", "svr_ncc_set_source",
     "svr_ncc_evaluate", "svr_ncc_alloc_targets", "svr_pyr_upload", "svr_pyr_level", "svr_nmi_bin_source", "svr_nmi_evaluate", "svr_stack_motion", "svr_slice_quality", "svr_correct_bias", "svr_normalise_bias", "svr_normalise_bias_local",
     "svr_normalise_bias_finish", "svr_init_reg_storage_volumes", "svr_fill_reg_slices",
     "svr_update_resampled_slices_i2w", "svr_prepare_slice_to_volume_reg", "svr_register_slices_to_volume",
@@ -482,6 +482,25 @@
         self._ck(self._lib.svr_unit_counts(self._h, o))
         return dict(pixels=int(o[0]), live_units=int(o[1]), dead_units=int(o[2]))
 
+    def coeff_kept_quads(self):
+        o = (C.c_uint64 * 3)()
+        self._ck(self._lib.svr_coeff_kept_quads(self._h, o))
+        return dict(kept_quads=int(o[0]), stored_units=int(o[1]), table_units=int(o[2]))
+
+    def coeff_read_unit(self, pid, plane):
+        out = np.empty((4, 16, 4), dtype=np.float32)
+        self._ck(self._lib.svr_coeff_read_unit(self._h, C.c_uint32(int(pid)), C.c_int(int(plane)), _p(out)))
+        return out
+
+    def coeff_read_pixels(self, idx, dense=True):
+        idx = np.ascontiguousarray(idx, dtype=np.uint32)
+        n = idx.size
+        pid = np.empty(n, dtype=np.uint32)
+        keep = np.empty((n, 16), dtype=np.uint64)
+        d = np.empty((n, 16, 4, 16, 4), dtype=np.float32) if dense else None
+        self._ck(self._lib.svr_coeff_read_pixels(self._h, _p(idx), C.c_uint32(n), _p(pid), _p(keep), _p(d) if dense else None))
+        return pid, keep, d
+
     def slab_chunks(self, world, rank):
         a, b = C.c_size_t(0), C.c_size_t(0)
         self._ck(self._lib.svr_slab_plan(self._h, int(world), int(rank), C.byref(a), C.byref(b)))
diff --git a/include/svr_hip.h b/include/svr_hip.h
--- a/include/svr_hip.h
+++ b/include/svr_hip.h
@@ -168,6 +168,9 @@
 int svr_timer_enable(svr_ctx *ctx, int enable);
 int svr_counters(svr_ctx *ctx, uint64_t out8[8]);
 int svr_unit_counts(svr_ctx *ctx, uint64_t out3[3]);
+int svr_coeff_kept_quads(svr_ctx *ctx, uint64_t out3[3]);
+int svr_coeff_read_unit(svr_ctx *ctx, uint32_t pid, int plane, float out[256]);
+int svr_coeff_read_pixels(svr_ctx *ctx, const uint32_t *idx, uint32_t n, uint32_t *pid, uint64_t *keep, float *dense);
 int svr_slice_em_setup(svr_ctx *ctx, int ns_global, int world, int rank, const int *rank_lo, const int *order_or_null, double step);
 int svr_slice_em_set_state(svr_ctx *ctx, const float *slice_weights_global, const unsigned char *excluded_global, const double scalars5[5],
                            const float em3[3]);
```

After: 203.0. -7.5%, worse.
